# CFGpp-diffusion/CFGpp

Measured on AMD Instinct MI355X. Metric: images/sec, higher is better.
Workload: dtype fp16; 1 GPU; SD1.5 512x512 ddim_cfg++ 50 NFE lambda=0.6 batch=8/GPU; per_gpu_batch=8, global_batch=8, nfe=50, unet_batch_rows=16, weights=seeded synthetic, exact diffusers shapes, build_id=cfgpp-build:d24daf2249552bfd:nogit

## Files before the change

### cfgpp_amd/_lib.py

```python
from __future__ import annotations

import ctypes as C
import os

HERE = os.path.dirname(os.path.abspath(__file__))
LIB_PATH = os.environ.get("CFGPP_LIB") or os.path.join(HERE, "libcfgpp_hip.so")


class CfgppError(RuntimeError):
    pass


class UNetConfigC(C.Structure):
    _fields_ = [
        ("in_channels", C.c_int), ("out_channels", C.c_int),
        ("num_levels", C.c_int),
        ("block_out_channels", C.c_int * 4),
        ("layers_per_block", C.c_int),
        ("level_has_attn", C.c_int * 4),
        ("transformer_depth", C.c_int * 4),
        ("num_heads", C.c_int * 4),
        ("cross_attention_dim", C.c_int),
        ("addition_embed", C.c_int),
        ("addition_time_embed_dim", C.c_int),
        ("addition_pooled_dim", C.c_int),
        ("norm_groups", C.c_int),
        ("sample_h", C.c_int), ("sample_w", C.c_int),
        ("max_rows", C.c_int),
    ]


_P, _I, _F, _L = C.c_void_p, C.c_int, C.c_float, C.c_long

PROTOTYPES = {
    "cfgpp_last_error": (C.c_char_p, []),
    "cfgpp_build_id": (C.c_char_p, []),
    "cfgpp_step_ddim": (_I, [_P, _P, _P, _P, _I, _F, _F, _F, _F, _F, _I, _I, _L, _P]),
    "cfgpp_step_ddim_h": (_I, [_P, _P, _P, _P, _F, _F, _F, _F, _F, _I, _I, _L, _P]),
    "cfgpp_step_ddim_masked": (_I, [_P, _P, _P, _P, _F, _F, _F, _F, _F, _I, _I, _P, _P, _P, _F, _F, _I, _L, _P]),
    "cfgpp_kdiff_input": (_I, [_P, _P, _F, _I, _L, _P]),
    "cfgpp_step_kdiff": (_I, [_P, _P, _P, _P, _P, C.POINTER(C.c_float), _I, _I, _I, _I, _L, _P]),
    "cfgpp_kdiff_denoise": (_I, [_P, _P, _P, _F, _F, _P, _P, _L, _P]),
    "cfgpp_lincomb": (_I, [_P, _P, _P, _P, _F, _F, _I, _L, _P]),
    "cfgpp_unet_create": (_P, [C.POINTER(UNetConfigC), _I]),
    "cfgpp_unet_destroy": (None, [_P]),
    "cfgpp_unet_load_tensor": (_I, [_P, C.c_char_p, _P, _I, C.POINTER(C.c_long), _I]),
    "cfgpp_unet_missing": (_I, [_P]),
    "cfgpp_unet_finalize": (_I, [_P]),
    "cfgpp_unet_set_context": (_I, [_P, _P, _I, _I, _P, _P, _I, _P]),
    "cfgpp_unet_image_condition": (_I, [_P, _P, _I, _P]),
    "cfgpp_unet_forward": (_I, [_P, _P, _I, _I, _F, _P, _I, _P]),
    "cfgpp_sample_graph_ddim": (_I, [_P, _P, _P, _I, _I, _P, _P, _P, _I, C.POINTER(C.c_float), _I, _F, _I, _I, _P]),
    "cfgpp_unet_profile": (_I, [_P, _P, _I, _I, _F, _P, _I, _P, C.POINTER(C.c_double), C.POINTER(C.c_double), C.POINTER(C.c_int), C.c_char_p, _L]),
    "cfgpp_unet_tuning": (_I, [_P, _I, C.POINTER(C.c_int), _I, _I]),
    "cfgpp_unet_attach_control": (_I, [_P, _P, _F]),
    "cfgpp_unet_flops": (C.c_double, [_P, _I]),
    "cfgpp_unet_device_bytes": (C.c_double, [_P]),
    "cfgpp_vae_create": (_P, [_I, _I, _I, _F, _I]),
    "cfgpp_vae_destroy": (None, [_P]),
    "cfgpp_vae_load_tensor": (_I, [_P, C.c_char_p, _P, _I, C.POINTER(C.c_long), _I]),
    "cfgpp_vae_finalize": (_I, [_P]),
    "cfgpp_vae_decode": (_I, [_P, _P, _P, _I, _P]),
    "cfgpp_vae_decode_image": (_I, [_P, _P, _P, _I, _P]),
    "cfgpp_vae_encode": (_I, [_P, _P, _P, _P, _P, _I, _P]),
    "cfgpp_vae_profile": (_I, [_P, _P, _P, _I, _P, C.c_char_p, C.c_long]),
    "cfgpp_vae_flops": (C.c_double, [_P, _I]),
    "cfgpp_text_create": (_P, [_I, _I, _I, _I, _I, _I, _I, _I, _I]),
    "cfgpp_text_destroy": (None, [_P]),
    "cfgpp_text_load_tensor": (_I, [_P, C.c_char_p, _P, _I, C.POINTER(C.c_long), _I]),
    "cfgpp_text_finalize": (_I, [_P]),
    "cfgpp_text_encode": (_I, [_P, C.POINTER(C.c_int), C.POINTER(C.c_int), _I, _I, _P, _P, _P]),
    "cfgpp_text_device_bytes": (C.c_double, [_P]),
    "cfgpp_vae_encode_flops": (C.c_double, [_P, _I]),
    "cfgpp_vae_device_bytes": (C.c_double, [_P]),
}

DEBUG_PROTOTYPES = {
    "cfgpp_op_softmax_rows": (_I, [_P, _L, _I, _P]),
    "cfgpp_op_conv_in_ex": (_I, [_P, _I, _P, _P, _P, _I, _I, _I, _I, _I, _I, _P, _P, _F, _P]),
    "cfgpp_op_groupnorm": (_I, [_P, _P, _P, _P, _P, _P, _I, _I, _I, _I, _I, _I, _F, _I, _I, _P]),
    "cfgpp_op_groupnorm_pre": (_I, [_P, _P, _P, _P, _P, _P, _P, _P, _I, _I, _I, _I, _I, _I, _F, _I, _I, _P]),
    "cfgpp_op_igemm_set_gstat": (None, [_P]),
    "cfgpp_op_igemm_gstat_written": (_I, []),
    "cfgpp_groupnorm_set_prestats": (None, [_I]),
    "cfgpp_groupnorm_prestats_enabled": (_I, []),
    "cfgpp_op_layernorm": (_I, [_P, _P, _P, _P, _L, _I, _F, _P]),
    "cfgpp_op_attention_prepare_vt": (_I, [_P, _I, _I, _I, _P]),
    "cfgpp_op_attention": (_I, [_P, _P, _P, _P, _I, _I, _I, _I, _I, _I, _I, _P]),
    "cfgpp_op_conv_in": (_I, [_P, _I, _P, _P, _P, _I, _I, _I, _I, _I, _I, _P]),
    "cfgpp_op_conv_in_cond": (_I, [_P, _I, _P, _I, _I, _P, _P, _P, _I, _I, _I, _I, _I, _I, _P]),
    "cfgpp_op_conv_in_add": (_I, [_P, _I, _P, _I, _I, _P, _I, _P, _P, _P, _I, _I, _I, _I, _I, _I, _P]),
    "cfgpp_op_cn_conv3x3": (_I, [_P, _I, _P, _I, _P, _P, _I, _I, _I, _I, _I, _I, _I, _P]),
    "cfgpp_op_residual_add": (_I, [C.POINTER(C.c_void_p), C.POINTER(C.c_void_p), C.POINTER(C.c_int), _I, _I, _F, _P]),
    "cfgpp_op_residual_nchw": (_I, [_P, _P, _I, _I, _I, _I, _F, _P]),
    "cfgpp_controlnet_residual": (_I, [_P, _I, _F, _P, _I, C.POINTER(C.c_int), _P]),
    "cfgpp_op_vae_posterior": (_I, [_P, _P, _P, _P, _P, _P, _I, _I, _F, _P]),
    "cfgpp_op_conv_out": (_I, [_P, _P, _I, _P, _P, _I, _I, _I, _I, _I, _P]),
    "cfgpp_op_conv_out_ex": (_I, [_P, _P, _I, _P, _P, _I, _I, _I, _I, _I, _F, _F, _I, _P]),
    "cfgpp_conv_out_set_tiled": (None, [_I]),
    "cfgpp_op_sinusoid": (_I, [_P, _F, _P, _I, _I, _I, _I, _P]),
    "cfgpp_op_skinny_gemm": (_I, [_P, _I, _P, _P, _P, _I, _P, _I, _I, _I, _I, _I, _I, _P]),
    "cfgpp_op_f16_to_f32_rows": (_I, [_P, _P, _I, _I, _I, _I, _P]),
    "cfgpp_op_igemm": (_I, [_P, _P, _I, _I, _I, _I, _I, _I, _P, _I, _I, _P, _P, _I, _P, _I, _I, _P, _I, _I, _I, _P]),
    "cfgpp_op_igemm_heads": (_I, [_P, _I, _P, _I, _I, _P, _I, _P, _P, _P, _I, _I, _I, _I, _I, _I, _P]),
    "cfgpp_igemm_force_config": (None, [_I]),
    "cfgpp_igemm_set_staging": (None, [_I]),
    "cfgpp_igemm_set_staged_epilogue": (None, [_I]),
    "cfgpp_igemm_set_big_tiles": (None, [_I]),
    "cfgpp_igemm_set_tail_split": (None, [_I]),
    "cfgpp_igemm_set_autotune": (None, [_I]),
    "cfgpp_igemm_set_blocked_walk": (None, [_I]),
    "cfgpp_igemm_walk_plan_probe": (None, [_I, _I, _I, _I, _I, _I, _I, C.POINTER(C.c_int)]),
    "cfgpp_igemm_set_n_major": (None, [_I]),
    "cfgpp_igemm_force_split": (None, [_I]),
    "cfgpp_igemm_set_split_tile": (None, [_I]),
    "cfgpp_igemm_set_mf16": (None, [_I]),
    "cfgpp_igemm_set_mf16_rounds": (None, [_I]),
    "cfgpp_igemm_set_mf16_heads": (None, [_I]),
    "cfgpp_igemm_set_mf16_linear": (None, [_I]),
    "cfgpp_igemm_set_big_split": (None, [_I]),
    "cfgpp_igemm_set_tune_mask": (None, [C.c_uint]),
    "cfgpp_igemm_tuner_state": (C.c_uint, []),
    "cfgpp_igemm_timeline": (None, [_P, _L, _I]),
    "cfgpp_igemm_timeline_info": (None, [C.POINTER(C.c_int)]),
    "cfgpp_groupnorm_set_mode": (None, [_I]),
    "cfgpp_layernorm_set_rows_per_wave": (None, [_I]),
    "cfgpp_attention_set_dma": (None, [_I]),
    "cfgpp_attention_set_stagger": (None, [_I]),
    "cfgpp_attention_set_cross": (None, [_I]),
}

_lib = None


def load():
    global _lib
    if _lib is not None:
        return _lib
    if not os.path.exists(LIB_PATH):
        raise CfgppError(
            f"{LIB_PATH} not found: build it with `python -m cfgpp_amd.build` "
            "(__graft_entry__.build()).  The HIP path has no CPU fallback.")
    import torch
    try:
        lib = C.CDLL(LIB_PATH)
    except OSError as e:
        raise CfgppError(f"cannot load {LIB_PATH}: {e}") from e
    for name, (res, args) in list(PROTOTYPES.items()) + list(DEBUG_PROTOTYPES.items()):
        try:
            fn = getattr(lib, name)
        except AttributeError as e:
            raise CfgppError(f"{LIB_PATH} does not export {name}") from e
        fn.restype = res
        fn.argtypes = args
    if os.environ.get("CFGPP_AUTOTUNE", "1") == "0":
        lib.cfgpp_igemm_set_autotune(0)
    _lib = lib
    return lib


def build_id() -> str:
    return load().cfgpp_build_id().decode("utf-8", "replace")


def last_error() -> str:
    return load().cfgpp_last_error().decode("utf-8", "replace")


def check(rc: int, what: str):
    if rc != 0:
        raise CfgppError(f"{what} failed (rc={rc}): {last_error()}")
```

### cfgpp_amd/csrc/cfgpp_debug.h

```cpp
#ifndef CFGPP_DEBUG_H
#define CFGPP_DEBUG_H
#ifdef __cplusplus
extern "C" {
#endif

int cfgpp_op_softmax_rows(void* s, long rows, int ncols, void* stream);
int cfgpp_op_conv_in_ex(const void* z, int z_is_half, void* out, const float* w, const float* bias,
                        int R, int zB, int Cin, int H, int W, int Cout, const float* pre_w, const float* pre_b,
                        float in_scale, void* stream);
int cfgpp_op_groupnorm(const void* src0, const void* src1, void* dst, const float* gamma, const float* beta,
                       float* stats, int N, int H, int W, int C0, int C1, int G, float eps, int silu,
                       int dst_padded, void* stream);
int cfgpp_op_groupnorm_pre(const void* src0, const void* src1, void* dst, const float* gamma, const float* beta,
                           const float* gst0, const float* gst1, float* stats, int N, int H, int W, int C0, int C1, int G,
                           float eps, int silu, int dst_padded, void* stream);
void cfgpp_op_igemm_set_gstat(void* buf);
int cfgpp_op_igemm_gstat_written(void);
void cfgpp_groupnorm_set_prestats(int on);
int cfgpp_groupnorm_prestats_enabled(void);
void cfgpp_groupnorm_set_mode(int mode);
int cfgpp_op_layernorm(const void* x, void* y, const float* gamma, const float* beta, long rows, int C,
                       float eps, void* stream);
void cfgpp_layernorm_set_rows_per_wave(int rpw);
int cfgpp_op_attention_prepare_vt(void* vt, int BH, int d, int tok_pad, void* stream);
int cfgpp_op_attention(const void* q, const void* k, const void* vt, void* o, int B, int heads, int d,
                       int nq, int nk, int q_tok_pad, int k_tok_pad, void* stream);
void cfgpp_attention_set_dma(int mode);
void cfgpp_attention_set_stagger(int sleeps);
void cfgpp_attention_set_cross(int on);
int cfgpp_op_conv_in(const void* z, int z_is_half, void* out, const float* w, const float* bias,
                     int R, int zB, int Cin, int H, int W, int Cout, void* stream);
int cfgpp_op_conv_in_cond(const void* z, int z_is_half, const void* cond, int cond_rows, int Cc, void* out, const float* w,
                          const float* bias, int R, int zB, int Cz, int H, int W, int Cout, void* stream);
int cfgpp_op_conv_in_add(const void* z, int z_is_half, const void* cond, int cond_rows, int Cc, const void* addend, int add_rows,
                         void* out, const float* w, const float* bias, int R, int zB, int Cz, int H, int W, int Cout, void* stream);
int cfgpp_op_cn_conv3x3(const void* in, int in_kind, void* out, int out_pad, const float* w, const float* bias, int R, int Ci, int Co,
                        int Hi, int Wi, int stride, int silu, void* stream);
int cfgpp_op_residual_add(void* const* dst, const void* const* src, const int* hwc, int n, int rows, float scale, void* stream);
int cfgpp_op_residual_nchw(const void* src, float* out, int rows, int H, int W, int C, float scale, void* stream);
int cfgpp_controlnet_residual(cfgpp_unet* cn, int i, float scale, float* out, int rows, int* hwc_out, void* stream);

int cfgpp_op_vae_posterior(const float* conv_out, const float* qw, const float* qb, const float* noise, float* z,
                           float* moments, int B, int HW, float scale, void* stream);
int cfgpp_op_conv_out(const void* x, void* out, int out_is_half, const void* w, const float* bias,
                      int R, int H, int W, int C, int Cout, void* stream);
int cfgpp_op_conv_out_ex(const void* x, void* out, int out_is_half, const void* w, const float* bias,
                         int R, int H, int W, int C, int Cout, float post_scale, float post_shift, int clamp01, void* stream);
void cfgpp_conv_out_set_tiled(int on);
int cfgpp_op_sinusoid(const float* vals, float scalar, float* out, int count, int dim, int out_ld, int out_off,
                      void* stream);
int cfgpp_op_skinny_gemm(const float* x, int ldx, const void* w, const float* bias, const float* addend, int add_ld,
                         float* out, int ldo, int M, int N, int K, int silu_in, int silu_out, void* stream);
int cfgpp_op_f16_to_f32_rows(const void* in, float* out, int rows, int cols, int out_ld, int out_off, void* stream);

int cfgpp_op_igemm(const void* a0, const void* a1, int C0, int C1, int taps, int amode, int H, int W,
                   const void* w, int M, int N, const float* bias, const float* temb, int temb_ld,
                   const void* resid, int rmode, int rld, void* out, int omode, int old_, int epi,
                   void* stream);
int cfgpp_op_igemm_heads(const void* a, int K, const void* w, int M, int N, const float* bias, int rows_per_batch,
                         void* hq, void* hk, void* hvt, int part0, int part_width, int head_dim, int heads,
                         int q_tok_pad, int tok_pad, void* stream);
void cfgpp_igemm_force_config(int cfg);
void cfgpp_igemm_set_tail_split(int on);
void cfgpp_igemm_set_mf16(int mode);
void cfgpp_igemm_set_mf16_linear(int on);
void cfgpp_igemm_set_mf16_heads(int on);
void cfgpp_igemm_set_mf16_rounds(int n);
void cfgpp_igemm_set_split_tile(int cfg);
void cfgpp_igemm_force_split(int s);
void cfgpp_igemm_set_big_split(int min_kt);
void cfgpp_igemm_set_n_major(int mode);
void cfgpp_igemm_set_blocked_walk(int on);
void cfgpp_igemm_walk_plan_probe(int M, int N, int K, int BM, int BN, int smem, int n_major, int* out5);
void cfgpp_igemm_set_tune_mask(unsigned mask);
unsigned cfgpp_igemm_tuner_state(void);
void cfgpp_igemm_set_autotune(int on);
void cfgpp_igemm_set_big_tiles(int on);
void cfgpp_igemm_set_staged_epilogue(int on);
void cfgpp_igemm_set_staging(int glds);
void cfgpp_igemm_timeline(void* buf, long cap_blocks, int target);
void cfgpp_igemm_timeline_info(int* out12);

#ifdef __cplusplus
}
#endif
#endif
```

### cfgpp_amd/csrc/common.h

```cpp
#pragma once
#include <hip/hip_runtime.h>
#include <stdint.h>

typedef _Float16 half_t;
typedef _Float16 half2_t __attribute__((ext_vector_type(2)));
typedef _Float16 half4_t __attribute__((ext_vector_type(4)));
typedef _Float16 half8_t __attribute__((ext_vector_type(8)));
typedef float f32x4 __attribute__((ext_vector_type(4)));
typedef float f32x16 __attribute__((ext_vector_type(16)));

#define CFGPP_WAVE 64

void cfgpp_set_error(const char* fmt, ...);
int cfgpp_claim_device(int device_id);
#define CFGPP_HIP_CHECK(expr)                                                         \
    do {                                                                              \
        hipError_t _e = (expr);                                                       \
        if (_e != hipSuccess) {                                                       \
            cfgpp_set_error("%s:%d: %s -> %s", __FILE__, __LINE__, #expr,             \
                            hipGetErrorString(_e));                                   \
            return -1;                                                                \
        }                                                                             \
    } while (0)
#define CFGPP_REQUIRE(cond, ...)                                                      \
    do {                                                                              \
        if (!(cond)) {                                                                \
            cfgpp_set_error(__VA_ARGS__);                                             \
            return -2;                                                                \
        }                                                                             \
    } while (0)

int step_advance_launch(const float* tab, int* idx, float* cur, hipStream_t s);
int step_ddim_dev_launch(void* z, void* z0t_out, const void* eps_uc, const void* eps_c, int eps_is_half, int z_is_half, float lam,
                         const float* cdev, int tweedie_uc, int renoise_uc, long n, hipStream_t s);

struct CnAddEntry {
    half_t* dst;
    const half_t* src;
    int H, W, C, pad_;
};
int cn_residual_add_launch(const CnAddEntry* tab, int n, long max_n8, int rows, float scale, hipStream_t s);

static inline int cdiv(long a, long b) { return (int)((a + b - 1) / b); }

struct RowMap {
    int mode;
    int H, W;
    int ld;
};

__host__ __device__ __forceinline__ int cfgpp_vt_pos(int tok) {
    return (tok & ~12) | ((tok & 4) << 1) | ((tok & 8) >> 1);
}

__device__ __forceinline__ float silu_f(float x) { return x / (1.0f + __expf(-x)); }
__device__ __forceinline__ float gelu_erf_f(float x) {
    const float ax = fabsf(x) * 0.70710678118654752440f;
    const float t = __builtin_amdgcn_rcpf(1.0f + 0.3275911f * ax);
    const float poly = t * (0.254829592f + t * (-0.284496736f + t * (1.421413741f + t * (-1.453152027f + t * 1.061405429f))));
    const float erfc_ax = poly * __builtin_amdgcn_exp2f(-ax * ax * 1.4426950408889634f);
    const float cdf = x >= 0.f ? 1.0f - 0.5f * erfc_ax : 0.5f * erfc_ax;
    return x * cdf;
}

typedef float f32x2 __attribute__((ext_vector_type(2)));
#define CFGPP_GELU_C 4.75f
#define CFGPP_GELU_POLY {4.912262559e-01f, 5.645360425e-02f, -1.591939032e-01f, 2.464362979e-01f, -1.982378513e-01f, 1.363233291e-02f, \
                         1.386516690e-01f, -1.158297956e-01f, -9.092462249e-03f, 6.090912968e-02f, -1.936562732e-02f, -1.160200126e-02f, \
                         6.012340542e-03f}
__device__ __forceinline__ f32x2 gelu_erf_pk(f32x2 x) {
    constexpr float k[13] = CFGPP_GELU_POLY;
    f32x2 a;
    a.x = fminf(fabsf(x.x), CFGPP_GELU_C); a.y = fminf(fabsf(x.y), CFGPP_GELU_C);
    const f32x2 t = __builtin_elementwise_fma(a, (f32x2){2.0f / CFGPP_GELU_C, 2.0f / CFGPP_GELU_C}, (f32x2){-1.0f, -1.0f});
    f32x2 p = {k[12], k[12]};
#pragma unroll
    for (int i = 11; i >= 0; --i) p = __builtin_elementwise_fma(p, t, (f32x2){k[i], k[i]});
    f32x2 m;
    m.x = fabsf(x.x) * p.x; m.y = fabsf(x.y) * p.y;
    return __builtin_elementwise_fma(x, (f32x2){0.5f, 0.5f}, m);
}

template <int MAXV>
__device__ __forceinline__ void ln_row_stats(const half8_t (&raw)[MAXV], int chunks, int C, float eps, int lane,
                                             float (&v)[MAXV][8], float& mean, float& rstd) {
    float sum = 0.f;
#pragma unroll
    for (int j = 0; j < MAXV; ++j) {
        const bool live = lane + j * 64 < chunks;
#pragma unroll
        for (int k = 0; k < 8; ++k) { v[j][k] = live ? (float)raw[j][k] : 0.f; sum += v[j][k]; }
    }
#pragma unroll
    for (int o = 32; o > 0; o >>= 1) sum += __shfl_xor(sum, o);
    mean = sum / (float)C;
    float sq = 0.f;
#pragma unroll
    for (int j = 0; j < MAXV; ++j) {
        const bool live = lane + j * 64 < chunks;
#pragma unroll
        for (int k = 0; k < 8; ++k) { const float d = v[j][k] - mean; sq += live ? d * d : 0.f; }
    }
#pragma unroll
    for (int o = 32; o > 0; o >>= 1) sq += __shfl_xor(sq, o);
    rstd = rsqrtf(sq / (float)C + eps);
}
__device__ __forceinline__ half8_t ln_row_affine(const float (&v)[8], float mean, float rstd, const float4 (&g)[2], const float4 (&be)[2]) {
    const float gg[8] = {g[0].x, g[0].y, g[0].z, g[0].w, g[1].x, g[1].y, g[1].z, g[1].w};
    const float bb[8] = {be[0].x, be[0].y, be[0].z, be[0].w, be[1].x, be[1].y, be[1].z, be[1].w};
    half8_t o;
#pragma unroll
    for (int k = 0; k < 8; ++k) o[k] = (half_t)((v[k] - mean) * rstd * gg[k] + bb[k]);
    return o;
}
```

### cfgpp_amd/csrc/engine_base.h

```cpp
#pragma once
#include <algorithm>
#include <cmath>
#include <cstring>
#include <deque>
#include <functional>
#include <map>
#include <string>
#include <vector>

#include "../../include/cfgpp.h"
#include "cfgpp_debug.h"
#include "igemm.h"

namespace {


struct HostParam {
    std::vector<long> shape;
    std::vector<half_t> h;
    std::vector<float> f;
    bool is_matrix = false;
    bool loaded = false;
    long numel() const { long n = 1; for (long s : shape) n *= s; return n; }
};

struct Tensor {
    half_t* p = nullptr;
    int H = 0, W = 0, C = 0;
    float* gst = nullptr;
    int* gst_ok = nullptr;
};

using Op = std::function<int(hipStream_t, int )>;


struct EngineBase {
    int max_rows = 1;
    int norm_groups = 32;
    std::map<std::string, HostParam> params;
    std::vector<void*> allocs;
    double dev_bytes = 0;
    double macs_per_row = 0;
    double attn_macs_per_row = 0;

    std::vector<Op> plan;
    std::vector<int> plan_kind;
    std::vector<double> plan_macs;
    std::vector<std::string> plan_desc;
    void tag(int kind, double macs, const std::string& desc = "") {
        plan_kind.resize(plan.size(), 3); plan_macs.resize(plan.size(), 0.0); plan_desc.resize(plan.size());
        if (!plan.empty()) { plan_kind.back() = kind; plan_macs.back() = macs; plan_desc.back() = desc; }
    }
    std::deque<int> cfg_hints;
    std::vector<int*> plan_hint;
    int tuned_rows = 0;
    std::map<int, std::vector<int>> tuned_by_rows;
    int* new_hint(bool in_main_plan) {
        cfg_hints.push_back(0);
        int* h = &cfg_hints.back();
        if (in_main_plan) { plan_hint.resize(plan.size() + 1, nullptr); plan_hint[plan.size()] = h; }
        return h;
    }
    int tune_plan(hipStream_t s, int rows) {
        auto cached = tuned_by_rows.find(rows);
        if (cached != tuned_by_rows.end() && cached->second.size() == cfg_hints.size()) {
            size_t k = 0;
            for (int& h : cfg_hints) h = cached->second[k++];
            tuned_rows = rows;
            return 0;
        }
        static const int cands[] = {0, 1, 4, 5, 6, 7, 8, 9, 10, 11, 12, 13, 14, 15, 16, 17, 20, 24, 25, 26, 27, 28};
        const size_t n = plan.size();
        plan_hint.resize(n, nullptr);
        hipStreamCaptureStatus cap = hipStreamCaptureStatusNone;
        if (hipStreamIsCapturing(s, &cap) != hipSuccess || cap != hipStreamCaptureStatusNone) return 0;
        std::vector<hipEvent_t> ev(n + 1, nullptr);
        for (auto& e : ev) if (hipEventCreate(&e) != hipSuccess) return -1;
        std::vector<float> base(n, 1e30f), best(n, 1e30f), t(n);
        std::vector<char> applied(n, 1);
        std::vector<int> bestc(n, 0);
        int rc = 0;
        auto timed_passes = [&]() {
            std::fill(t.begin(), t.end(), 1e30f);
            for (int rep = 0; rep < 2 && rc == 0; ++rep) {
                if (hipEventRecord(ev[0], s) != hipSuccess) rc = -1;
                for (size_t i = 0; i < n && rc == 0; ++i) {
                    rc = plan[i](s, rows);
                    if (plan_hint[i]) applied[i] = (char)igemm_last_hint_applied();
                    if (rc == 0 && hipEventRecord(ev[i + 1], s) != hipSuccess) rc = -1;
                }
                if (rc == 0 && hipEventSynchronize(ev[n]) != hipSuccess) rc = -1;
                for (size_t i = 0; i < n && rc == 0; ++i) {
                    if (!plan_hint[i]) continue;
                    float ms = 0.f;
                    if (hipEventElapsedTime(&ms, ev[i], ev[i + 1]) == hipSuccess && ms < t[i]) t[i] = ms;
                }
            }
        };
        const unsigned mask = igemm_tune_mask();
        for (int c : cands) {
            if (c != 0 && !((mask >> c) & 1u)) continue;
            for (int& h : cfg_hints) h = c;
            timed_passes();
            for (size_t i = 0; i < n; ++i) {
                if (c == 0) base[i] = t[i];
                if (t[i] < best[i] && (c == 0 || applied[i])) { best[i] = t[i]; bestc[i] = c; }
            }
        }
        for (size_t i = 0; i < n; ++i)
            if (plan_hint[i] && !(bestc[i] != 0 && best[i] < 0.97f * base[i])) { bestc[i] = 0; best[i] = base[i]; }
        for (int walk = 1; walk <= 2 && rc == 0 && (mask >> 31); ++walk) {
            for (size_t i = 0; i < n; ++i) if (plan_hint[i]) *plan_hint[i] = (bestc[i] & 63) | (walk << 6);
            timed_passes();
            for (size_t i = 0; i < n; ++i)
                if (plan_hint[i] && t[i] < 0.97f * best[i]) { best[i] = t[i]; bestc[i] = (bestc[i] & 63) | (walk << 6); }
        }
        for (int& h : cfg_hints) h = 0;
        for (size_t i = 0; i < n; ++i) if (plan_hint[i]) *plan_hint[i] = bestc[i];
        for (auto& e : ev) hipEventDestroy(e);
        if (rc == 0) tuned_by_rows[rows] = std::vector<int>(cfg_hints.begin(), cfg_hints.end());
        tuned_rows = rows;
        return rc;
    }
    std::map<std::tuple<int, int, int>, std::vector<std::pair<half_t*, float*>>> pool;
    std::deque<int> gst_flags;
    float* d_gn_stats = nullptr;
    static constexpr long KSPLIT_WS_BYTES = 128L << 20;
    float* d_ksplit_ws = nullptr;
    float* ksplit_ws() {
        if (!d_ksplit_ws) d_ksplit_ws = (float*)dmalloc((size_t)KSPLIT_WS_BYTES, false);
        return d_ksplit_ws;
    }

    void* dmalloc(size_t bytes, bool zero = true) {
        void* p = nullptr;
        if (hipMalloc(&p, bytes) != hipSuccess) return nullptr;
        if (zero) hipMemset(p, 0, bytes);
        allocs.push_back(p);
        dev_bytes += (double)bytes;
        return p;
    }
    Tensor acq(int H, int W, int C) {
        auto key = std::make_tuple(H, W, C);
        auto& fl = pool[key];
        Tensor t; t.H = H; t.W = W; t.C = C;
        gst_flags.push_back(0);
        t.gst_ok = &gst_flags.back();
        if (!fl.empty()) { t.p = fl.back().first; t.gst = fl.back().second; fl.pop_back(); return t; }
        t.p = (half_t*)dmalloc((size_t)max_rows * (H + 2) * (W + 2) * C * sizeof(half_t));
        if (H * W >= 1024 && (H * W) % 32 == 0 && C % 8 == 0)
            t.gst = (float*)dmalloc((size_t)max_rows * (H * W / 32) * C * 2 * sizeof(float), false);
        return t;
    }
    void rel(const Tensor& t) { if (t.p) pool[std::make_tuple(t.H, t.W, t.C)].push_back(std::make_pair(t.p, t.gst)); }
    ~EngineBase() { for (void* p : allocs) hipFree(p); }
};

void expect(EngineBase* u, const std::string& key, std::vector<long> shape, bool matrix) {
    HostParam hp; hp.shape = std::move(shape); hp.is_matrix = matrix;
    u->params[key] = std::move(hp);
}
void expect_linear(EngineBase* u, const std::string& p, long out, long in, bool bias = true) {
    expect(u, p + ".weight", {out, in}, true);
    if (bias) expect(u, p + ".bias", {out}, false);
}
void expect_conv(EngineBase* u, const std::string& p, long out, long in, int k) {
    expect(u, p + ".weight", {out, in, k, k}, true);
    expect(u, p + ".bias", {out}, false);
}
void expect_norm(EngineBase* u, const std::string& p, long c) {
    expect(u, p + ".weight", {c}, false);
    expect(u, p + ".bias", {c}, false);
}
void expect_resnet(EngineBase* u, const std::string& p, long cin, long cout, long temb) {
    expect_norm(u, p + ".norm1", cin);
    expect_conv(u, p + ".conv1", cout, cin, 3);
    expect_linear(u, p + ".time_emb_proj", cout, temb);
    expect_norm(u, p + ".norm2", cout);
    expect_conv(u, p + ".conv2", cout, cout, 3);
    if (cin != cout) expect_conv(u, p + ".conv_shortcut", cout, cin, 1);
}
void expect_transformer(EngineBase* u, const std::string& p, long c, int depth, long cross) {
    expect_norm(u, p + ".norm", c);
    expect(u, p + ".proj_in.weight", {c, c}, true);  expect(u, p + ".proj_in.bias", {c}, false);
    expect(u, p + ".proj_out.weight", {c, c}, true); expect(u, p + ".proj_out.bias", {c}, false);
    for (int k = 0; k < depth; ++k) {
        const std::string b = p + ".transformer_blocks." + std::to_string(k);
        expect_norm(u, b + ".norm1", c); expect_norm(u, b + ".norm2", c); expect_norm(u, b + ".norm3", c);
        expect_linear(u, b + ".attn1.to_q", c, c, false); expect_linear(u, b + ".attn1.to_k", c, c, false);
        expect_linear(u, b + ".attn1.to_v", c, c, false); expect_linear(u, b + ".attn1.to_out.0", c, c, true);
        expect_linear(u, b + ".attn2.to_q", c, c, false); expect_linear(u, b + ".attn2.to_k", c, cross, false);
        expect_linear(u, b + ".attn2.to_v", c, cross, false); expect_linear(u, b + ".attn2.to_out.0", c, c, true);
        expect_linear(u, b + ".ff.net.0.proj", 8 * c, c, true);
        expect_linear(u, b + ".ff.net.2", c, 4 * c, true);
    }
}

struct Builder {
    EngineBase* u;
    bool ok = true;
    std::string err;

    HostParam* get(const std::string& key) {
        auto it = u->params.find(key);
        if (it == u->params.end() || !it->second.loaded) { ok = false; err = "missing parameter " + key; return nullptr; }
        return &it->second;
    }
    template <typename T>
    T* upload(const std::vector<T>& v) {
        T* d = (T*)u->dmalloc(v.size() * sizeof(T), false);
        if (!d) { ok = false; err = "hipMalloc failed"; return nullptr; }
        if (hipMemcpy(d, v.data(), v.size() * sizeof(T), hipMemcpyHostToDevice) != hipSuccess) { ok = false; err = "hipMemcpy failed"; }
        return d;
    }
    void drop(const std::string& key) { auto& p = u->params[key]; std::vector<half_t>().swap(p.h); std::vector<float>().swap(p.f); }

    float* f32(const std::string& key) {
        HostParam* p = get(key); if (!p) return nullptr;
        float* d = upload(p->f); drop(key); return d;
    }
    half_t* linear(const std::string& key) {
        HostParam* p = get(key); if (!p) return nullptr;
        half_t* d = upload(p->h); drop(key); return d;
    }
    half_t* conv3(const std::string& key) {
        HostParam* p = get(key); if (!p) return nullptr;
        const long O = p->shape[0], I = p->shape[1];
        std::vector<half_t> r((size_t)O * 9 * I);
        for (long o = 0; o < O; ++o)
            for (long i = 0; i < I; ++i)
                for (int t = 0; t < 9; ++t) r[(size_t)o * 9 * I + ((i >> 6) * 9 + t) * 64 + (i & 63)] = p->h[((size_t)o * I + i) * 9 + t];
        half_t* d = upload(r); drop(key); return d;
    }
    std::vector<half_t> concat_host(const std::vector<std::string>& keys) {
        std::vector<half_t> r;
        for (auto& k : keys) { HostParam* p = get(k); if (!p) return {}; r.insert(r.end(), p->h.begin(), p->h.end()); }
        for (auto& k : keys) drop(k);
        return r;
    }
    half_t* concat(const std::vector<std::string>& keys) {
        std::vector<half_t> r = concat_host(keys);
        return ok ? upload(r) : nullptr;
    }
    bool geglu_host(const std::string& pfx, long C, std::vector<half_t>& rw, std::vector<float>& rb) {
        HostParam* pw = get(pfx + ".weight"); HostParam* pb = get(pfx + ".bias");
        if (!pw || !pb) return false;
        const long F = 4 * C;
        rw.resize((size_t)2 * F * C); rb.resize((size_t)2 * F);
        for (long f = 0; f < F; ++f) {
            const long pv = (f / 32) * 64 + (f % 32), pg = pv + 32;
            std::memcpy(&rw[(size_t)pv * C], &pw->h[(size_t)f * C], C * sizeof(half_t));
            std::memcpy(&rw[(size_t)pg * C], &pw->h[(size_t)(F + f) * C], C * sizeof(half_t));
            rb[pv] = pb->f[f]; rb[pg] = pb->f[F + f];
        }
        drop(pfx + ".weight"); drop(pfx + ".bias");
        return true;
    }
    void geglu(const std::string& pfx, long C, half_t** w, float** b) {
        std::vector<half_t> rw; std::vector<float> rb;
        if (!geglu_host(pfx, C, rw, rb)) return;
        *w = upload(rw); *b = upload(rb);
    }
};

inline int round_up(int a, int b) { return (a + b - 1) / b * b; }

IGemmArgs base_args(EngineBase* u = nullptr) {
    IGemmArgs a; std::memset(&a, 0, sizeof(a)); a.out_scale = 1.0f; a.taps = 1;
    if (u) { a.ws_buf = u->ksplit_ws(); a.ws_bytes = a.ws_buf ? EngineBase::KSPLIT_WS_BYTES : 0; }
    return a;
}

struct Plan {
    EngineBase* u;
    Builder* B;
    std::vector<Op>* ops;

    void conv3x3(const Tensor& src, const Tensor& dst, const half_t* w, const float* bias, int amode,
                 const float* temb, int temb_ld, const Tensor* resid, int ashift = 0) {
        IGemmArgs a = base_args(u);
        a.a0 = src.p; a.C0 = src.C; a.taps = 9; a.amode = amode; a.ashift = ashift; a.H = dst.H; a.W = dst.W;
        a.w = w; a.N = dst.C; a.K = 9 * src.C; a.bias = bias; a.temb = temb; a.temb_ld = temb_ld;
        a.rows_per_batch = dst.H * dst.W;
        if (resid) { a.resid = resid->p; a.rmode = 1; a.rld = resid->C; }
        a.out = dst.p; a.omode = 1; a.old = dst.C; a.epi = EPI_STORE;
        a.gstat = dst.gst; a.stat_flag = dst.gst ? dst.gst_ok : nullptr;
        const int HW = dst.H * dst.W;
        u->macs_per_row += (double)HW * dst.C * 9.0 * src.C;
        int* hint = u->new_hint(ops == &u->plan);
        ops->push_back([a, HW, hint](hipStream_t s, int rows) mutable { IGemmArgs b = a; b.M = rows * HW; b.cfg_hint = *hint; return igemm_launch(b, s); });
        if (ops == &u->plan) u->tag(0, (double)HW * dst.C * 9.0 * src.C, "conv3x3 amode=" + std::to_string(amode) + " HW=" + std::to_string(HW) + " N=" + std::to_string(dst.C) + " K=" + std::to_string(9 * src.C) + (resid ? " +res" : "") + (temb ? " +temb" : ""));
    }
    void conv1x1(const Tensor& s0, const Tensor* s1, const Tensor& dst, const half_t* w, const float* bias) {
        IGemmArgs a = base_args(u);
        a.a0 = s0.p; a.C0 = s0.C; if (s1) { a.a1 = s1->p; a.C1 = s1->C; }
        a.amode = 1; a.H = dst.H; a.W = dst.W; a.w = w; a.N = dst.C; a.K = a.C0 + a.C1; a.bias = bias;
        a.rows_per_batch = dst.H * dst.W; a.out = dst.p; a.omode = 1; a.old = dst.C; a.epi = EPI_STORE;
        const int HW = dst.H * dst.W;
        u->macs_per_row += (double)HW * dst.C * a.K;
        int* hint = u->new_hint(ops == &u->plan);
        ops->push_back([a, HW, hint](hipStream_t s, int rows) mutable { IGemmArgs b = a; b.M = rows * HW; b.cfg_hint = *hint; return igemm_launch(b, s); });
        if (ops == &u->plan) u->tag(0, (double)HW * dst.C * a.K, "conv1x1 HW=" + std::to_string(HW) + " N=" + std::to_string(dst.C) + " K=" + std::to_string(a.K));
    }
    void linear(const half_t* A, int K, half_t* out, int N, const half_t* w, const float* bias, const half_t* resid,
                int tokens, int epi = EPI_STORE) {
        IGemmArgs a = base_args(u);
        a.a0 = A; a.C0 = K; a.amode = 0; a.w = w; a.N = N; a.K = K; a.bias = bias;
        a.resid = resid; a.rmode = 0; a.rld = N; a.out = out; a.omode = 0;
        a.old = (epi == EPI_GEGLU) ? N / 2 : N; a.epi = epi; a.rows_per_batch = tokens;
        u->macs_per_row += (double)tokens * N * K;
        int* hint = u->new_hint(ops == &u->plan);
        ops->push_back([a, tokens, hint](hipStream_t s, int rows) mutable { IGemmArgs b = a; b.M = rows * tokens; b.cfg_hint = *hint; return igemm_launch(b, s); });
        if (ops == &u->plan) u->tag(0, (double)tokens * N * K, std::string(epi == EPI_GEGLU ? "geglu" : "linear") + " HW=" + std::to_string(tokens) + " N=" + std::to_string(N) + " K=" + std::to_string(K) + (resid ? " +res" : ""));
    }
    void linear_to_padded(const half_t* A, int K, const Tensor& dst, const half_t* w, const float* bias, const Tensor& resid) {
        IGemmArgs a = base_args(u);
        a.a0 = A; a.C0 = K; a.amode = 0; a.H = dst.H; a.W = dst.W; a.w = w; a.N = dst.C; a.K = K; a.bias = bias;
        a.resid = resid.p; a.rmode = 1; a.rld = resid.C; a.out = dst.p; a.omode = 1; a.old = dst.C;
        a.epi = EPI_STORE; a.rows_per_batch = dst.H * dst.W;
        a.gstat = dst.gst; a.stat_flag = dst.gst ? dst.gst_ok : nullptr;
        const int HW = dst.H * dst.W;
        u->macs_per_row += (double)HW * dst.C * K;
        int* hint = u->new_hint(ops == &u->plan);
        ops->push_back([a, HW, hint](hipStream_t s, int rows) mutable { IGemmArgs b = a; b.M = rows * HW; b.cfg_hint = *hint; return igemm_launch(b, s); });
        if (ops == &u->plan) u->tag(0, (double)HW * dst.C * K, "proj_out HW=" + std::to_string(HW) + " N=" + std::to_string(dst.C) + " K=" + std::to_string(K));
    }
    void heads(const half_t* A, int K, const half_t* w, int N, int tokens, int part0, int C, int nheads,
               half_t* q, half_t* k, half_t* vt, int q_tok_pad, int tok_pad, bool count = true,
               const float* bias = nullptr) {
        IGemmArgs a = base_args(u);
        const int d = C / nheads;
        a.a0 = A; a.C0 = K; a.amode = 0; a.w = w; a.N = N; a.K = K; a.epi = EPI_HEADS;
        a.bias = bias;
        a.rows_per_batch = tokens; a.hq = q; a.hk = k; a.hvt = vt; a.part0 = part0; a.part_width = C;
        a.head_dim = d; a.head_dim_pad = round_up(d, 32); a.heads = nheads; a.tok_pad = tok_pad; a.q_tok_pad = q_tok_pad;
        if (count) u->macs_per_row += (double)tokens * N * K;
        int* hint = u->new_hint(ops == &u->plan);
        ops->push_back([a, tokens, hint](hipStream_t s, int rows) mutable { IGemmArgs b = a; b.M = rows * tokens; b.cfg_hint = *hint; return igemm_launch(b, s); });
        if (ops == &u->plan) u->tag(0, count ? (double)tokens * N * K : 0.0, "heads HW=" + std::to_string(tokens) + " N=" + std::to_string(N) + " K=" + std::to_string(K));
    }
    void groupnorm(const Tensor& s0, const Tensor* s1, half_t* dst, bool dst_padded, const float* g, const float* b,
                   float eps, bool silu) {
        EngineBase* uu = u;
        const half_t* p0 = s0.p; const half_t* p1 = s1 ? s1->p : nullptr;
        const int H = s0.H, W = s0.W, C0 = s0.C, C1 = s1 ? s1->C : 0, G = u->norm_groups;
        const float* gst0 = s0.gst; const float* gst1 = s1 ? s1->gst : nullptr;
        const int* ok0 = s0.gst_ok; const int* ok1 = s1 ? s1->gst_ok : nullptr;
        ops->push_back([=](hipStream_t s, int rows) {
            if (cfgpp_groupnorm_prestats_enabled() && gst0 && ok0 && *ok0 && (!p1 || (gst1 && ok1 && *ok1)))
                return cfgpp_op_groupnorm_pre(p0, p1, dst, g, b, gst0, gst1, uu->d_gn_stats, rows, H, W, C0, C1, G, eps, silu ? 1 : 0,
                                              dst_padded ? 1 : 0, s);
            return cfgpp_op_groupnorm(p0, p1, dst, g, b, uu->d_gn_stats, rows, H, W, C0, C1, G, eps, silu ? 1 : 0,
                                      dst_padded ? 1 : 0, s);
        });
        if (ops == &u->plan) u->tag(2, 0.0, "groupnorm HW=" + std::to_string(H * W) + " C=" + std::to_string(C0 + C1));
    }
    void layernorm(const half_t* x, half_t* y, const float* g, const float* b, int tokens, int C) {
        ops->push_back([=](hipStream_t s, int rows) { return cfgpp_op_layernorm(x, y, g, b, (long)rows * tokens, C, 1e-5f, s); });
        if (ops == &u->plan) u->tag(2, 0.0, "layernorm HW=" + std::to_string(tokens) + " C=" + std::to_string(C));
    }
    void attention(const half_t* q, const half_t* k, const half_t* vt, half_t* o, int nheads, int d, int nq, int nk,
                   int q_tok_pad, int k_tok_pad) {
        u->attn_macs_per_row += 2.0 * (double)nheads * nq * nk * d;
        ops->push_back([=](hipStream_t s, int rows) {
            return cfgpp_op_attention(q, k, vt, o, rows, nheads, d, nq, nk, q_tok_pad, k_tok_pad, s);
        });
        if (ops == &u->plan) u->tag(1, 2.0 * (double)nheads * nq * nk * d, "self_attn heads=" + std::to_string(nheads) + " N=" + std::to_string(nq) + " d=" + std::to_string(d));
    }
};

}
```

### cfgpp_amd/csrc/small_kernels.hip

```cpp
#include "common.h"

namespace {

template <typename TIN>
__global__ void __launch_bounds__(256)
conv_in_kernel(const TIN* __restrict__ z, const half_t* __restrict__ cond, int Cc, int cond_rows,
               half_t* __restrict__ out, const float* __restrict__ w,
               const float* __restrict__ bias, int R, int zB, int Cz, int H, int W, int Cout,
               const float* __restrict__ pre_w, const float* __restrict__ pre_b, float in_scale,
               const half_t* __restrict__ add, int add_rows) {
    constexpr int TP = 16;
    __shared__ float patch[TP][9 * 16];
    const int r = blockIdx.y;
    const int p0 = blockIdx.x * TP;
    const int HW = H * W;
    const int zb = r % zB;
    const int cb = cond ? zb % cond_rows : 0;
    const int Cin = Cz + Cc;
    const int K = 9 * Cin;
    for (int i = threadIdx.x; i < TP * K; i += blockDim.x) {
        const int tp = i / K, k = i - tp * K;
        const int tap = k / Cin, ci = k - tap * Cin;
        const int p = p0 + tp;
        float v = 0.f;
        if (p < HW) {
            const int y = p / W + tap / 3 - 1, x = p % W + tap % 3 - 1;
            if (y >= 0 && y < H && x >= 0 && x < W) {
                if (ci >= Cz) {
                    v = (float)cond[((long)(cb * Cc + ci - Cz) * H + y) * W + x];
                } else if (pre_w) {
                    float acc = pre_b ? pre_b[ci] : 0.f;
                    for (int j = 0; j < Cz; ++j)
                        acc += pre_w[ci * Cz + j] * (float)(half_t)((float)z[((long)(zb * Cz + j) * H + y) * W + x] * in_scale);
                    v = acc;
                } else {
                    v = (float)z[((long)(zb * Cz + ci) * H + y) * W + x] * in_scale;
                }
            }
        }
        patch[tp][k] = (float)(half_t)v;
    }
    __syncthreads();
    for (int co = threadIdx.x; co < Cout; co += blockDim.x) {
        float acc[TP];
        const float b = bias ? bias[co] : 0.f;
#pragma unroll
        for (int tp = 0; tp < TP; ++tp) acc[tp] = b;
        for (int k = 0; k < K; ++k) {
            const float wv = w[(long)k * Cout + co];
#pragma unroll
            for (int tp = 0; tp < TP; ++tp) acc[tp] += wv * patch[tp][k];
        }
#pragma unroll
        for (int tp = 0; tp < TP; ++tp) {
            const int p = p0 + tp;
            if (p < HW) {
                const int y = p / W, x = p - y * W;
                half_t v = (half_t)acc[tp];
                if (add) v = (half_t)((float)v + (float)add[((long)((zb % add_rows) * (H + 2) + y + 1) * (W + 2) + x + 1) * Cout + co]);
                out[((long)(r * (H + 2) + y + 1) * (W + 2) + x + 1) * Cout + co] = v;
            }
        }
    }
}

template <int CO, typename TOUT>
__global__ void __launch_bounds__(256)
conv_out_kernel(const half_t* __restrict__ x, TOUT* __restrict__ out, const half_t* __restrict__ w,
                const float* __restrict__ bias, int R, int H, int W, int C, int cout_real,
                float post_scale, float post_shift, int clamp01) {
    const int lane = threadIdx.x & 63;
    const long pix = (long)blockIdx.x * 4 + (threadIdx.x >> 6);
    const long total = (long)R * H * W;
    if (pix >= total) return;
    const int HW = H * W;
    const int r = (int)(pix / HW), p = (int)(pix - (long)r * HW);
    const int y = p / W, xq = p - y * W;
    const int cpt = C / 8;
    float acc[CO];
#pragma unroll
    for (int o = 0; o < CO; ++o) acc[o] = 0.f;
    for (int c = lane; c < 9 * cpt; c += 64) {
        const int tap = c / cpt, cc = (c - tap * cpt) * 8;
        const int dy = tap / 3 - 1, dx = tap % 3 - 1;
        const half8_t xv = *reinterpret_cast<const half8_t*>(
            x + ((long)(r * (H + 2) + y + 1 + dy) * (W + 2) + xq + 1 + dx) * C + cc);
#pragma unroll
        for (int o = 0; o < CO; ++o) {
            const half8_t wv = *reinterpret_cast<const half8_t*>(w + ((long)o * 9 + tap) * C + cc);
#pragma unroll
            for (int k = 0; k < 8; ++k) acc[o] += (float)xv[k] * (float)wv[k];
        }
    }
#pragma unroll
    for (int o = 0; o < CO; ++o)
#pragma unroll
        for (int s = 32; s > 0; s >>= 1) acc[o] += __shfl_xor(acc[o], s);
    if (lane < cout_real) {
        float v = 0.f;
#pragma unroll
        for (int o = 0; o < CO; ++o) if (lane == o) v = acc[o];
        v += bias ? bias[lane] : 0.f;
        v = v * post_scale + post_shift;
        if (clamp01) v = fminf(fmaxf(v, 0.f), 1.f);
        out[((long)(r * cout_real + lane) * H + y) * W + xq] = (TOUT)v;
    }
}

template <int CO, typename TOUT>
__global__ void __launch_bounds__(256)
conv_out_tile_kernel(const half_t* __restrict__ x, TOUT* __restrict__ out, const half_t* __restrict__ w,
                     const float* __restrict__ bias, int R, int H, int W, int C, int cout_real,
                     float post_scale, float post_shift, int clamp01) {
    constexpr int TH = 8, TW = 32, HH = TH + 2, HW_ = TW + 2, PITCH = 144;
    __shared__ __attribute__((aligned(16))) char tile[HH * HW_ * PITCH];
    const int tid = threadIdx.x;
    const int tiles_x = (W + TW - 1) / TW, tiles_y = (H + TH - 1) / TH;
    int b = blockIdx.x;
    const int txi = b % tiles_x; b /= tiles_x;
    const int tyi = b % tiles_y; const int r = b / tiles_y;
    const int y0 = tyi * TH, x0 = txi * TW;
    const int ty = tid >> 5, tx = tid & 31;
    typedef _Float16 h2 __attribute__((ext_vector_type(2)));
    float acc[CO];
#pragma unroll
    for (int o = 0; o < CO; ++o) acc[o] = 0.f;
    const half_t* xr = x + (long)r * (H + 2) * (W + 2) * C;
    for (int cb = 0; cb < C; cb += 64) {
        __syncthreads();
        for (int i = tid; i < HH * HW_ * 8; i += 256) {
            const int px = i >> 3, ch = i & 7;
            const int hy = px / HW_, hx = px - hy * HW_;
            const int gy = y0 + hy, gx = x0 + hx;
            half8_t v = {0, 0, 0, 0, 0, 0, 0, 0};
            if (gy < H + 2 && gx < W + 2) v = *reinterpret_cast<const half8_t*>(xr + ((long)gy * (W + 2) + gx) * C + cb + ch * 8);
            *reinterpret_cast<half8_t*>(tile + px * PITCH + ch * 16) = v;
        }
        __syncthreads();
#pragma unroll
        for (int tap = 0; tap < 9; ++tap) {
            const int dy = tap / 3, dx = tap - 3 * (tap / 3);
            const char* px = tile + ((ty + dy) * HW_ + tx + dx) * PITCH;
#pragma unroll
            for (int ch = 0; ch < 8; ++ch) {
                const half8_t xv = *reinterpret_cast<const half8_t*>(px + ch * 16);
#pragma unroll
                for (int o = 0; o < CO; ++o) {
                    const half8_t wv = *reinterpret_cast<const half8_t*>(w + ((long)o * 9 + tap) * C + cb + ch * 8);
#pragma unroll
                    for (int k = 0; k < 4; ++k)
                        acc[o] = __builtin_amdgcn_fdot2((h2){xv[2 * k], xv[2 * k + 1]}, (h2){wv[2 * k], wv[2 * k + 1]}, acc[o], false);
                }
            }
        }
    }
    const int y = y0 + ty, xq = x0 + tx;
    if (y < H && xq < W) {
#pragma unroll
        for (int o = 0; o < CO; ++o) {
            if (o < cout_real) {
                float v = acc[o] + (bias ? bias[o] : 0.f);
                v = v * post_scale + post_shift;
                if (clamp01) v = fminf(fmaxf(v, 0.f), 1.f);
                out[((long)(r * cout_real + o) * H + y) * W + xq] = (TOUT)v;
            }
        }
    }
}

__global__ void sinusoid_kernel(const float* __restrict__ vals, float scalar, float* __restrict__ out,
                                int count, int dim, int out_ld, int out_off) {
    const int i = blockIdx.x;
    const int half_dim = dim / 2;
    const float v = vals ? vals[i] : scalar;
    for (int j = threadIdx.x; j < half_dim; j += blockDim.x) {
        const float e = expf(-9.210340371976184f * (float)j / (float)half_dim);
        const float arg = v * e;
        out[(long)i * out_ld + out_off + j] = (float)(half_t)cosf(arg);
        out[(long)i * out_ld + out_off + half_dim + j] = (float)(half_t)sinf(arg);
    }
}

template <int MB, int NB>
__global__ void __launch_bounds__(256)
skinny_gemm_kernel(const float* __restrict__ x, int ldx, const half_t* __restrict__ w, const float* __restrict__ bias,
                   const float* __restrict__ addend, int add_ld, float* __restrict__ out, int ldo,
                   int M, int N, int K, int silu_in, int silu_out) {
    const int lane = threadIdx.x & 63, wid = threadIdx.x >> 6;
    const int n0 = (blockIdx.x * 4 + wid) * NB;
    const int m0 = blockIdx.y * MB;
    if (n0 >= N) return;
    float acc[MB][NB];
#pragma unroll
    for (int i = 0; i < MB; ++i)
#pragma unroll
        for (int j = 0; j < NB; ++j) acc[i][j] = 0.f;
    for (int kc = lane * 8; kc < K; kc += 64 * 8) {
        float xv[MB][8];
#pragma unroll
        for (int i = 0; i < MB; ++i) {
            const int m = min(m0 + i, M - 1);
            const float4 a = *reinterpret_cast<const float4*>(x + (long)m * ldx + kc);
            const float4 b = *reinterpret_cast<const float4*>(x + (long)m * ldx + kc + 4);
            xv[i][0] = a.x; xv[i][1] = a.y; xv[i][2] = a.z; xv[i][3] = a.w;
            xv[i][4] = b.x; xv[i][5] = b.y; xv[i][6] = b.z; xv[i][7] = b.w;
            if (silu_in) {
#pragma unroll
                for (int k = 0; k < 8; ++k) xv[i][k] = silu_f(xv[i][k]);
            }
        }
#pragma unroll
        for (int j = 0; j < NB; ++j) {
            const int n = min(n0 + j, N - 1);
            const half8_t wv = *reinterpret_cast<const half8_t*>(w + (long)n * K + kc);
#pragma unroll
            for (int i = 0; i < MB; ++i)
#pragma unroll
                for (int k = 0; k < 8; ++k) acc[i][j] += xv[i][k] * (float)wv[k];
        }
    }
#pragma unroll
    for (int i = 0; i < MB; ++i)
#pragma unroll
        for (int j = 0; j < NB; ++j)
#pragma unroll
            for (int s = 32; s > 0; s >>= 1) acc[i][j] += __shfl_xor(acc[i][j], s);
    if (lane == 0) {
#pragma unroll
        for (int i = 0; i < MB; ++i) {
            const int m = m0 + i;
            if (m >= M) continue;
#pragma unroll
            for (int j = 0; j < NB; ++j) {
                const int n = n0 + j;
                if (n >= N) continue;
                float v = acc[i][j] + (bias ? bias[n] : 0.f);
                if (addend) v += addend[(long)m * add_ld + n];
                if (silu_out) v = silu_f(v);
                out[(long)m * ldo + n] = v;
            }
        }
    }
}

__global__ void f16_to_f32_rows_kernel(const half_t* __restrict__ in, float* __restrict__ out, int rows, int cols,
                                       int out_ld, int out_off) {
    const long n = (long)rows * cols;
    for (long i = (long)blockIdx.x * blockDim.x + threadIdx.x; i < n; i += (long)gridDim.x * blockDim.x) {
        const int r = (int)(i / cols), c = (int)(i - (long)r * cols);
        out[(long)r * out_ld + out_off + c] = (float)in[i];
    }
}

}


__global__ void __launch_bounds__(256)
vae_posterior_kernel(const float* __restrict__ co, const float* __restrict__ qw, const float* __restrict__ qb,
                     const float* __restrict__ noise, float* __restrict__ z, float* __restrict__ moments,
                     int B, int HW, float scale) {
    const long i = (long)blockIdx.x * blockDim.x + threadIdx.x;
    if (i >= (long)B * HW) return;
    const int b = (int)(i / HW), p = (int)(i - (long)b * HW);
    float x[8], m[8];
#pragma unroll
    for (int j = 0; j < 8; ++j) x[j] = (float)(half_t)co[((long)b * 8 + j) * HW + p];
#pragma unroll
    for (int o = 0; o < 8; ++o) {
        float acc = qb[o];
#pragma unroll
        for (int j = 0; j < 8; ++j) acc += qw[o * 8 + j] * x[j];
        m[o] = (float)(half_t)acc;
    }
#pragma unroll
    for (int c = 0; c < 4; ++c) {
        const float lv = fminf(fmaxf(m[4 + c], -30.f), 20.f);
        const float n = noise ? noise[((long)b * 4 + c) * HW + p] : 0.f;
        z[((long)b * 4 + c) * HW + p] = (m[c] + __expf(0.5f * lv) * n) * scale;
        if (moments) { moments[((long)b * 8 + c) * HW + p] = m[c]; moments[((long)b * 8 + 4 + c) * HW + p] = lv; }
    }
}

extern "C" {

int cfgpp_op_vae_posterior(const float* conv_out, const float* qw, const float* qb, const float* noise, float* z,
                           float* moments, int B, int HW, float scale, void* stream) {
    CFGPP_REQUIRE(conv_out && qw && qb && z && B > 0 && HW > 0, "vae_posterior: bad args");
    hipLaunchKernelGGL(vae_posterior_kernel, dim3(cdiv((long)B * HW, 256)), dim3(256), 0, (hipStream_t)stream, conv_out, qw, qb, noise, z, moments, B, HW, scale);
    CFGPP_HIP_CHECK(hipGetLastError());
    return 0;
}

int cfgpp_op_conv_in_add(const void* z, int z_is_half, const void* cond, int cond_rows, int Cc, const void* addend, int add_rows,
                         void* out, const float* w, const float* bias, int R, int zB, int Cz, int H, int W, int Cout, void* stream);

int cfgpp_op_conv_in_cond(const void* z, int z_is_half, const void* cond, int cond_rows, int Cc, void* out, const float* w,
                          const float* bias, int R, int zB, int Cz, int H, int W, int Cout, void* stream) {
    return cfgpp_op_conv_in_add(z, z_is_half, cond, cond_rows, Cc, nullptr, 1, out, w, bias, R, zB, Cz, H, W, Cout, stream);
}

int cfgpp_op_conv_in_add(const void* z, int z_is_half, const void* cond, int cond_rows, int Cc, const void* addend, int add_rows,
                         void* out, const float* w, const float* bias, int R, int zB, int Cz, int H, int W, int Cout, void* stream) {
    CFGPP_REQUIRE(Cz >= 1 && Cz <= 8, "conv_in: Cin=%d (<= 8)", Cz);
    CFGPP_REQUIRE(!addend || add_rows > 0, "conv_in: addend with add_rows=%d", add_rows);
    const half_t* add = (const half_t*)addend;
    if (!add) add_rows = 1;
    CFGPP_REQUIRE(!cond || (Cc >= 1 && Cz + Cc <= 16 && cond_rows > 0), "conv_in: condition of %d channels x %d rows on %d latent channels (Cin <= 16)",
                  Cc, cond_rows, Cz);
    CFGPP_REQUIRE(z && out && w && R > 0 && zB > 0, "conv_in: bad args");
    if (!cond) { Cc = 0; cond_rows = 1; }
    dim3 grid(cdiv((long)H * W, 16), R);
    hipStream_t s = (hipStream_t)stream;
    if (z_is_half)
        hipLaunchKernelGGL(conv_in_kernel<half_t>, grid, dim3(256), 0, s, (const half_t*)z, (const half_t*)cond, Cc, cond_rows, (half_t*)out, w, bias,
                           R, zB, Cz, H, W, Cout, (const float*)nullptr, (const float*)nullptr, 1.0f, add, add_rows);
    else
        hipLaunchKernelGGL(conv_in_kernel<float>, grid, dim3(256), 0, s, (const float*)z, (const half_t*)cond, Cc, cond_rows, (half_t*)out, w, bias,
                           R, zB, Cz, H, W, Cout, (const float*)nullptr, (const float*)nullptr, 1.0f, add, add_rows);
    CFGPP_HIP_CHECK(hipGetLastError());
    return 0;
}

int cfgpp_op_conv_in_ex(const void* z, int z_is_half, void* out, const float* w, const float* bias,
                        int R, int zB, int Cin, int H, int W, int Cout, const float* pre_w, const float* pre_b,
                        float in_scale, void* stream) {
    CFGPP_REQUIRE(Cin >= 1 && Cin <= 8, "conv_in: Cin=%d (<= 8)", Cin);
    CFGPP_REQUIRE(z && out && w && R > 0 && zB > 0, "conv_in: bad args");
    dim3 grid(cdiv((long)H * W, 16), R);
    hipStream_t s = (hipStream_t)stream;
    if (z_is_half)
        hipLaunchKernelGGL(conv_in_kernel<half_t>, grid, dim3(256), 0, s, (const half_t*)z, (const half_t*)nullptr, 0, 1, (half_t*)out, w, bias,
                           R, zB, Cin, H, W, Cout, pre_w, pre_b, in_scale, (const half_t*)nullptr, 1);
    else
        hipLaunchKernelGGL(conv_in_kernel<float>, grid, dim3(256), 0, s, (const float*)z, (const half_t*)nullptr, 0, 1, (half_t*)out, w, bias,
                           R, zB, Cin, H, W, Cout, pre_w, pre_b, in_scale, (const half_t*)nullptr, 1);
    CFGPP_HIP_CHECK(hipGetLastError());
    return 0;
}

int cfgpp_op_conv_in(const void* z, int z_is_half, void* out, const float* w, const float* bias,
                     int R, int zB, int Cin, int H, int W, int Cout, void* stream) {
    return cfgpp_op_conv_in_ex(z, z_is_half, out, w, bias, R, zB, Cin, H, W, Cout, nullptr, nullptr, 1.0f, stream);
}

int cfgpp_op_conv_out_ex(const void* x, void* out, int out_is_half, const void* w, const float* bias,
                         int R, int H, int W, int C, int Cout, float post_scale, float post_shift, int clamp01, void* stream);
static int g_conv_out_tiled = 1;
void cfgpp_conv_out_set_tiled(int on) { g_conv_out_tiled = on ? 1 : 0; }

int cfgpp_op_conv_out(const void* x, void* out, int out_is_half, const void* w, const float* bias,
                      int R, int H, int W, int C, int Cout, void* stream) {
    return cfgpp_op_conv_out_ex(x, out, out_is_half, w, bias, R, H, W, C, Cout, 1.0f, 0.0f, 0, stream);
}

int cfgpp_op_conv_out_ex(const void* x, void* out, int out_is_half, const void* w, const float* bias,
                         int R, int H, int W, int C, int Cout, float post_scale, float post_shift, int clamp01, void* stream) {
    CFGPP_REQUIRE(Cout >= 1 && Cout <= 8 && C % 8 == 0, "conv_out: Cout=%d C=%d", Cout, C);
    CFGPP_REQUIRE(x && out && w, "conv_out: null pointer");
    const long total = (long)R * H * W;
    dim3 grid(cdiv(total, 4));
    hipStream_t s = (hipStream_t)stream;
    if (Cout <= 4 && C % 64 == 0 && (long)H * W >= 128 * 128 && g_conv_out_tiled) {
        dim3 tg((unsigned)((long)R * cdiv(H, 8) * cdiv(W, 32)));
        if (out_is_half)
            hipLaunchKernelGGL((conv_out_tile_kernel<4, half_t>), tg, dim3(256), 0, s, (const half_t*)x, (half_t*)out, (const half_t*)w, bias, R, H, W, C, Cout, post_scale, post_shift, clamp01);
        else if (Cout <= 3)
            hipLaunchKernelGGL((conv_out_tile_kernel<3, float>), tg, dim3(256), 0, s, (const half_t*)x, (float*)out, (const half_t*)w, bias, R, H, W, C, Cout, post_scale, post_shift, clamp01);
        else
            hipLaunchKernelGGL((conv_out_tile_kernel<4, float>), tg, dim3(256), 0, s, (const half_t*)x, (float*)out, (const half_t*)w, bias, R, H, W, C, Cout, post_scale, post_shift, clamp01);
        CFGPP_HIP_CHECK(hipGetLastError());
        return 0;
    }
    if (Cout > 4) {
        CFGPP_REQUIRE(!out_is_half, "conv_out: 8-channel output is fp32 only");
        hipLaunchKernelGGL((conv_out_kernel<8, float>), grid, dim3(256), 0, s, (const half_t*)x, (float*)out, (const half_t*)w, bias, R, H, W, C, Cout, post_scale, post_shift, clamp01);
    } else if (out_is_half)
        hipLaunchKernelGGL((conv_out_kernel<4, half_t>), grid, dim3(256), 0, s, (const half_t*)x, (half_t*)out, (const half_t*)w, bias, R, H, W, C, Cout, post_scale, post_shift, clamp01);
    else
        hipLaunchKernelGGL((conv_out_kernel<4, float>), grid, dim3(256), 0, s, (const half_t*)x, (float*)out, (const half_t*)w, bias, R, H, W, C, Cout, post_scale, post_shift, clamp01);
    CFGPP_HIP_CHECK(hipGetLastError());
    return 0;
}

int cfgpp_op_sinusoid(const float* vals, float scalar, float* out, int count, int dim, int out_ld, int out_off,
                      void* stream) {
    CFGPP_REQUIRE(out && count > 0 && dim % 2 == 0, "sinusoid: bad args");
    hipLaunchKernelGGL(sinusoid_kernel, dim3(count), dim3(128), 0, (hipStream_t)stream, vals, scalar, out, count, dim, out_ld, out_off);
    CFGPP_HIP_CHECK(hipGetLastError());
    return 0;
}

int cfgpp_op_skinny_gemm(const float* x, int ldx, const void* w, const float* bias, const float* addend, int add_ld,
                         float* out, int ldo, int M, int N, int K, int silu_in, int silu_out, void* stream) {
    CFGPP_REQUIRE(x && w && out && M > 0 && N > 0 && K % 8 == 0, "skinny_gemm: bad args (K=%d)", K);
    hipStream_t s = (hipStream_t)stream;
    if (M == 1) {
        dim3 grid(cdiv(N, 4 * 2), 1);
        hipLaunchKernelGGL((skinny_gemm_kernel<1, 2>), grid, dim3(256), 0, s, x, ldx, (const half_t*)w, bias, addend, add_ld, out, ldo, M, N, K, silu_in, silu_out);
    } else {
        dim3 grid(cdiv(N, 4 * 2), cdiv(M, 4));
        hipLaunchKernelGGL((skinny_gemm_kernel<4, 2>), grid, dim3(256), 0, s, x, ldx, (const half_t*)w, bias, addend, add_ld, out, ldo, M, N, K, silu_in, silu_out);
    }
    CFGPP_HIP_CHECK(hipGetLastError());
    return 0;
}

int cfgpp_op_f16_to_f32_rows(const void* in, float* out, int rows, int cols, int out_ld, int out_off, void* stream) {
    hipLaunchKernelGGL(f16_to_f32_rows_kernel, dim3(cdiv((long)rows * cols, 256) > 1024 ? 1024 : cdiv((long)rows * cols, 256)),
                       dim3(256), 0, (hipStream_t)stream, (const half_t*)in, out, rows, cols, out_ld, out_off);
    CFGPP_HIP_CHECK(hipGetLastError());
    return 0;
}

}
```

### cfgpp_amd/csrc/unet.hip

```cpp
#include "engine_base.h"

struct cfgpp_unet : EngineBase {
    cfgpp_unet_config cfg;
    int device = 0;
    bool finalized = false;

    std::vector<Op> ctx_plan;
    const void* in_z = nullptr; int in_z_half = 0; int in_z_rows = 0; float in_t = 0.f; void* out_eps = nullptr;
    const float* in_t_dev = nullptr;
    half_t* d_cond = nullptr; int cond_rows = 0;
    float* d_step_tab = nullptr; int step_tab_cap = 0; float* d_step_cur = nullptr; int* d_step_idx = nullptr;
    hipStream_t cap_stream = nullptr;
    struct GraphKey { const void* z; void* z0t; void* eps; const void* euc; const void* ec; int z_half, z_rows, rows, tw, rn; float lam; long n; int tuned_serial; int cond_rows; };
    struct Graph { GraphKey key; hipGraph_t graph; hipGraphExec_t exec; };
    std::vector<Graph> graphs;
    int tuned_serial = 0;
    static void destroy(Graph& g) { if (g.exec) hipGraphExecDestroy(g.exec); if (g.graph) hipGraphDestroy(g.graph); g.exec = nullptr; g.graph = nullptr; }
    void drop_graphs() { for (auto& g : graphs) destroy(g); graphs.clear(); }
    ~cfgpp_unet() { drop_graphs(); if (cap_stream) hipStreamDestroy(cap_stream); }
    const half_t* ctx_ehs = nullptr; int ctx_rows = 0; int ctx_tokens = 77;
    const half_t* ctx_text = nullptr; const float* ctx_tids = nullptr; int ctx_cond_rows = 0;
    bool ctx_set = false;

    float* d_sin_t = nullptr; float* d_emb_h = nullptr; float* d_emb_t = nullptr; float* d_emb = nullptr;
    float* d_temb_all = nullptr; int temb_total = 0;
    float* d_add_in = nullptr; float* d_add_h = nullptr; float* d_aug = nullptr;

    half_t *tok_x = nullptr, *tok_ln = nullptr, *tok_attn = nullptr, *tok_ff = nullptr;
    half_t *hq[4] = {nullptr, nullptr, nullptr, nullptr}, *hk[4] = {nullptr, nullptr, nullptr, nullptr},
           *hvt[4] = {nullptr, nullptr, nullptr, nullptr};

    bool control = false;
    std::vector<int> embed_ch;
    std::vector<Op> img_plan;
    const void* img_in = nullptr; int img_in_half = 0;
    half_t* d_img_emb = nullptr; int img_rows = 0;
    std::vector<Tensor> ctrl_res;
    std::vector<Tensor> ctrl_dst;
    cfgpp_unet* ctrl = nullptr; float ctrl_scale = 0.f;
    CnAddEntry* d_ctrl_tab = nullptr; long ctrl_max_n8 = 0;
};

namespace {

void build_param_table(cfgpp_unet* u) {
    const cfgpp_unet_config& c = u->cfg;
    const int L = c.num_levels;
    const long c0 = c.block_out_channels[0], temb = 4 * c0;
    expect_conv(u, "conv_in", c0, c.in_channels, 3);
    expect_linear(u, "time_embedding.linear_1", temb, c0);
    expect_linear(u, "time_embedding.linear_2", temb, temb);
    if (c.addition_embed) {
        const long in = (long)c.addition_time_embed_dim * 6 + c.addition_pooled_dim;
        expect_linear(u, "add_embedding.linear_1", temb, in);
        expect_linear(u, "add_embedding.linear_2", temb, temb);
    }
    long ch = c0;
    for (int i = 0; i < L; ++i) {
        const long co = c.block_out_channels[i];
        const std::string p = "down_blocks." + std::to_string(i);
        for (int j = 0; j < c.layers_per_block; ++j) {
            expect_resnet(u, p + ".resnets." + std::to_string(j), ch, co, temb);
            if (c.level_has_attn[i])
                expect_transformer(u, p + ".attentions." + std::to_string(j), co, c.transformer_depth[i], c.cross_attention_dim);
            ch = co;
        }
        if (i != L - 1) expect_conv(u, p + ".downsamplers.0.conv", co, co, 3);
    }
    const long cm = c.block_out_channels[L - 1];
    expect_resnet(u, "mid_block.resnets.0", cm, cm, temb);
    expect_transformer(u, "mid_block.attentions.0", cm, c.transformer_depth[L - 1], c.cross_attention_dim);
    expect_resnet(u, "mid_block.resnets.1", cm, cm, temb);
    if (u->control) {
        const std::vector<int>& e = u->embed_ch;
        const std::string q = "controlnet_cond_embedding.";
        expect_conv(u, q + "conv_in", e[0], 3, 3);
        for (size_t i = 0; i + 1 < e.size(); ++i) {
            expect_conv(u, q + "blocks." + std::to_string(2 * i), e[i], e[i], 3);
            expect_conv(u, q + "blocks." + std::to_string(2 * i + 1), e[i + 1], e[i], 3);
        }
        expect_conv(u, q + "conv_out", c0, e.back(), 3);
        int k = 0;
        expect_conv(u, "controlnet_down_blocks." + std::to_string(k++), c0, c0, 1);
        for (int i = 0; i < L; ++i) {
            const long co = c.block_out_channels[i];
            for (int j = 0; j < c.layers_per_block; ++j) expect_conv(u, "controlnet_down_blocks." + std::to_string(k++), co, co, 1);
            if (i != L - 1) expect_conv(u, "controlnet_down_blocks." + std::to_string(k++), co, co, 1);
        }
        expect_conv(u, "controlnet_mid_block", cm, cm, 1);
        return;
    }
    long prev = cm;
    for (int i = 0; i < L; ++i) {
        const int lvl = L - 1 - i;
        const long co = c.block_out_channels[lvl];
        const long cin_lvl = c.block_out_channels[std::max(lvl - 1, 0)];
        const std::string p = "up_blocks." + std::to_string(i);
        for (int j = 0; j < c.layers_per_block + 1; ++j) {
            const long skip = (j == c.layers_per_block) ? cin_lvl : co;
            const long rin = (j == 0 ? prev : co) + skip;
            expect_resnet(u, p + ".resnets." + std::to_string(j), rin, co, temb);
            if (c.level_has_attn[lvl])
                expect_transformer(u, p + ".attentions." + std::to_string(j), co, c.transformer_depth[lvl], c.cross_attention_dim);
        }
        if (i != L - 1) expect_conv(u, p + ".upsamplers.0.conv", co, co, 3);
        prev = co;
    }
    expect_norm(u, "conv_norm_out", c0);
    expect_conv(u, "conv_out", c.out_channels, c0, 3);
}

struct ResW {
    float *n1g, *n1b, *n2g, *n2b, *b1, *b2, *bsc;
    half_t *w1, *w2, *wsc;
    int temb_off;
    int cin, cout;
};

int controlnet_tail(cfgpp_unet* u, Builder& B, Plan& P, const std::vector<Tensor>& skips, const Tensor& mid) {
    const cfgpp_unet_config& c = u->cfg;
    const int R = c.max_rows, c0 = c.block_out_channels[0];
    auto persist = [&](int H, int W, int C) {
        Tensor t; t.H = H; t.W = W; t.C = C;
        t.p = (half_t*)u->dmalloc((size_t)R * (H + 2) * (W + 2) * C * sizeof(half_t));
        return t;
    };
    for (size_t k = 0; k <= skips.size(); ++k) {
        const Tensor& src = k < skips.size() ? skips[k] : mid;
        const std::string key = k < skips.size() ? "controlnet_down_blocks." + std::to_string(k) : std::string("controlnet_mid_block");
        half_t* w = B.linear(key + ".weight"); float* b = B.f32(key + ".bias");
        Tensor r = persist(src.H, src.W, src.C);
        CFGPP_REQUIRE(r.p, "finalize: hipMalloc failed");
        P.conv1x1(src, nullptr, r, w, b);
        u->ctrl_res.push_back(r);
    }
    const std::vector<int>& e = u->embed_ch;
    const int n = (int)e.size();
    const std::string q = "controlnet_cond_embedding.";
    struct Layer { std::string key; int ci, co, stride; };
    std::vector<Layer> layers;
    layers.push_back({q + "conv_in", 3, e[0], 1});
    for (int i = 0; i + 1 < n; ++i) {
        layers.push_back({q + "blocks." + std::to_string(2 * i), e[i], e[i], 1});
        layers.push_back({q + "blocks." + std::to_string(2 * i + 1), e[i], e[i + 1], 2});
    }
    long scratch = 1;
    {
        int h = c.sample_h << (n - 1), w = c.sample_w << (n - 1);
        for (size_t l = 0; l + 1 < layers.size(); ++l) {
            if (layers[l].stride == 2) { h = (h - 1) / 2 + 1; w = (w - 1) / 2 + 1; }
            scratch = std::max(scratch, (long)R * h * w * layers[l].co);
        }
    }
    half_t* buf[2] = {(half_t*)u->dmalloc((size_t)scratch * sizeof(half_t), false), (half_t*)u->dmalloc((size_t)scratch * sizeof(half_t), false)};
    Tensor pre = persist(c.sample_h, c.sample_w, e.back());
    CFGPP_REQUIRE(buf[0] && buf[1] && pre.p, "finalize: hipMalloc failed");
    cfgpp_unet* uu = u;
    int h = c.sample_h << (n - 1), w = c.sample_w << (n - 1);
    for (size_t l = 0; l < layers.size(); ++l) {
        const Layer& ly = layers[l];
        HostParam* pw = B.get(ly.key + ".weight");
        CFGPP_REQUIRE(pw, "finalize: %s", B.err.c_str());
        std::vector<float> r((size_t)9 * ly.ci * ly.co);
        for (int o = 0; o < ly.co; ++o) for (int i = 0; i < ly.ci; ++i) for (int t = 0; t < 9; ++t)
            r[((size_t)t * ly.ci + i) * ly.co + o] = (float)pw->h[((size_t)o * ly.ci + i) * 9 + t];
        B.drop(ly.key + ".weight");
        float* dw = B.upload(r); float* db = B.f32(ly.key + ".bias");
        const bool last = l + 1 == layers.size();
        const half_t* in = l == 0 ? nullptr : buf[(l - 1) & 1];
        half_t* out = last ? pre.p : buf[l & 1];
        const int hi = h, wi = w, ci = ly.ci, co = ly.co, st = ly.stride, first = l == 0;
        u->img_plan.push_back([=](hipStream_t s, int rows) {
            return cfgpp_op_cn_conv3x3(first ? uu->img_in : in, first ? (uu->img_in_half ? 1 : 2) : 0, out, last ? 1 : 0, dw, db, rows, ci,
                                       co, hi, wi, st, 1, s);
        });
        if (st == 2) { h = (h - 1) / 2 + 1; w = (w - 1) / 2 + 1; }
    }
    CFGPP_REQUIRE(h == c.sample_h && w == c.sample_w, "finalize: internal error, the embedding ends at %d x %d", h, w);
    {
        half_t* wo = B.conv3(q + "conv_out.weight"); float* bo = B.f32(q + "conv_out.bias");
        Tensor dst; dst.p = u->d_img_emb; dst.H = c.sample_h; dst.W = c.sample_w; dst.C = c0;
        Plan PI{u, &B, &u->img_plan};
        const double macs = u->macs_per_row;
        PI.conv3x3(pre, dst, wo, bo, 1, nullptr, 0, nullptr);
        u->macs_per_row = macs;
    }
    CFGPP_REQUIRE(B.ok, "finalize: %s", B.err.c_str());
    return 0;
}

}

extern "C" {

static cfgpp_unet* unet_new(const cfgpp_unet_config* cfg, int device_id, const int* embed, int n_embed) {
    if (!cfg) { cfgpp_set_error("unet_create: null config"); return nullptr; }
    if (cfg->num_levels < 1 || cfg->num_levels > 4 || cfg->layers_per_block < 1 || cfg->max_rows < 1) {
        cfgpp_set_error("unet_create: bad config"); return nullptr;
    }
    for (int i = 0; i < cfg->num_levels; ++i) {
        const int c = cfg->block_out_channels[i];
        if (c % 64 != 0 || c % cfg->norm_groups != 0) { cfgpp_set_error("unet_create: channels %d must be a multiple of 64 and of norm_groups", c); return nullptr; }
        if (cfg->level_has_attn[i]) {
            const int d = c / cfg->num_heads[i];
            if (c % cfg->num_heads[i] != 0 || d % 4 != 0 || d > 160) { cfgpp_set_error("unet_create: head dim %d unsupported", d); return nullptr; }
        }
    }
    if (cfg->cross_attention_dim % 64 != 0) { cfgpp_set_error("unet_create: cross_attention_dim must be a multiple of 64"); return nullptr; }
    if (!embed && cfg->in_channels > cfg->out_channels && cfg->in_channels > 16) {
        cfgpp_set_error("unet_create: in_channels=%d out_channels=%d (an inpaint UNet takes at most 16 input channels)", cfg->in_channels,
                        cfg->out_channels);
        return nullptr;
    }
    if ((cfg->sample_h % (1 << (cfg->num_levels - 1))) || (cfg->sample_w % (1 << (cfg->num_levels - 1)))) {
        cfgpp_set_error("unet_create: sample size must be divisible by 2^(levels-1)"); return nullptr;
    }
    int ndev = 0;
    if (hipGetDeviceCount(&ndev) != hipSuccess || ndev <= device_id) {
        cfgpp_set_error("unet_create: no HIP device %d (found %d) - the HIP path has no CPU fallback", device_id, ndev);
        return nullptr;
    }
    if (cfgpp_claim_device(device_id)) return nullptr;
    if (hipSetDevice(device_id) != hipSuccess) { cfgpp_set_error("unet_create: hipSetDevice failed"); return nullptr; }
    cfgpp_unet* u = new cfgpp_unet();
    u->cfg = *cfg; u->device = device_id; u->max_rows = cfg->max_rows; u->norm_groups = cfg->norm_groups;
    if (embed) { u->control = true; u->embed_ch.assign(embed, embed + n_embed); }
    build_param_table(u);
    return u;
}

cfgpp_unet* cfgpp_unet_create(const cfgpp_unet_config* cfg, int device_id) {
    if (cfg && cfg->out_channels == 0) {
        static const int embed[4] = {16, 32, 96, 256};
        if (cfg->in_channels < 1 || cfg->in_channels > 8) {
            cfgpp_set_error("unet_create: ControlNet (out_channels = 0) with in_channels=%d (1 .. 8 latent channels)", cfg->in_channels);
            return nullptr;
        }
        return unet_new(cfg, device_id, embed, 4);
    }
    return unet_new(cfg, device_id, nullptr, 0);
}


void cfgpp_unet_destroy(cfgpp_unet* u) {
    if (!u) return;
    delete u;
}

int cfgpp_unet_load_tensor(cfgpp_unet* u, const char* key, const void* host, int dtype, const long* shape, int ndim) {
    CFGPP_REQUIRE(u && key && host && shape, "load_tensor: null argument");
    CFGPP_REQUIRE(!u->finalized, "load_tensor: context already finalized");
    auto it = u->params.find(key);
    if (it == u->params.end()) { cfgpp_set_error("load_tensor: unknown key %s", key); return -3; }
    HostParam& p = it->second;
    long n = 1; for (int i = 0; i < ndim; ++i) n *= shape[i];
    CFGPP_REQUIRE(n == p.numel(), "load_tensor: %s has %ld elements, expected %ld", key, n, p.numel());
    if (ndim == 4) { p.shape.assign(shape, shape + 4); }
    if (p.is_matrix && !(std::string(key) == "conv_in.weight")) {
        p.h.resize(n);
        if (dtype == 0) { const float* s = (const float*)host; for (long i = 0; i < n; ++i) p.h[i] = (half_t)s[i]; }
        else std::memcpy(p.h.data(), host, n * sizeof(half_t));
    } else {
        p.f.resize(n);
        if (dtype == 0) std::memcpy(p.f.data(), host, n * sizeof(float));
        else { const half_t* s = (const half_t*)host; for (long i = 0; i < n; ++i) p.f[i] = (float)s[i]; }
    }
    p.loaded = true;
    return 0;
}

int cfgpp_unet_missing(cfgpp_unet* u) {
    if (!u) return -1;
    int n = 0; std::string names;
    for (auto& kv : u->params) if (!kv.second.loaded) { if (n < 8) names += kv.first + " "; ++n; }
    if (n) cfgpp_set_error("missing %d parameters: %s...", n, names.c_str());
    return n;
}

int cfgpp_unet_finalize(cfgpp_unet* u) {
    CFGPP_REQUIRE(u, "finalize: null");
    CFGPP_REQUIRE(!u->finalized, "finalize: already finalized");
    if (cfgpp_unet_missing(u) != 0) { const std::string m = cfgpp_last_error(); cfgpp_set_error("finalize: %s", m.c_str()); return -2; }
    CFGPP_HIP_CHECK(hipSetDevice(u->device));
    const cfgpp_unet_config& c = u->cfg;
    const int L = c.num_levels, R = c.max_rows;
    const int c0 = c.block_out_channels[0], temb_dim = 4 * c0;
    Builder B{u};
    Plan P{u, &B, &u->plan};
    Plan PC{u, &B, &u->ctx_plan};

    long max_tok_c = 0, max_ff = 0;
    {
        int H = c.sample_h, W = c.sample_w;
        for (int i = 0; i < L; ++i) {
            const long C = c.block_out_channels[i];
            if (c.level_has_attn[i] || i == L - 1) {
                const long tok = (long)H * W;
                const int d = (int)(C / c.num_heads[i]), dp = round_up(d, 32);
                max_tok_c = std::max(max_tok_c, tok * C);
                max_ff = std::max(max_ff, tok * 4 * C);
                u->hq[i] = (half_t*)u->dmalloc((size_t)R * c.num_heads[i] * round_up((int)tok, 128) * dp * 2);
                u->hk[i] = (half_t*)u->dmalloc((size_t)R * c.num_heads[i] * round_up((int)tok, 128) * dp * 2);
                u->hvt[i] = (half_t*)u->dmalloc((size_t)R * c.num_heads[i] * dp * round_up((int)tok, 64) * 2);
                CFGPP_REQUIRE(u->hq[i] && u->hk[i] && u->hvt[i], "finalize: hipMalloc failed");
                if (cfgpp_op_attention_prepare_vt(u->hvt[i], R * c.num_heads[i], d, round_up((int)tok, 64), nullptr)) return -1;
            }
            if (i != L - 1) { H /= 2; W /= 2; }
        }
    }
    u->tok_x = (half_t*)u->dmalloc((size_t)R * max_tok_c * 2);
    u->tok_ln = (half_t*)u->dmalloc((size_t)R * max_tok_c * 2);
    u->tok_attn = (half_t*)u->dmalloc((size_t)R * max_tok_c * 2);
    u->tok_ff = (half_t*)u->dmalloc((size_t)R * max_ff * 2);
    u->d_gn_stats = (float*)u->dmalloc((size_t)R * (1024 * 64 * 2 + 64 * 2) * sizeof(float));
    u->d_sin_t = (float*)u->dmalloc((size_t)c0 * sizeof(float));
    u->d_emb_h = (float*)u->dmalloc((size_t)temb_dim * sizeof(float));
    u->d_emb_t = (float*)u->dmalloc((size_t)temb_dim * sizeof(float));
    u->d_emb = (float*)u->dmalloc((size_t)R * temb_dim * sizeof(float));
    CFGPP_REQUIRE(u->tok_x && u->tok_ln && u->tok_attn && u->tok_ff, "finalize: hipMalloc failed");

    std::vector<std::string> res_names;
    {
        for (int i = 0; i < L; ++i)
            for (int j = 0; j < c.layers_per_block; ++j) res_names.push_back("down_blocks." + std::to_string(i) + ".resnets." + std::to_string(j));
        res_names.push_back("mid_block.resnets.0"); res_names.push_back("mid_block.resnets.1");
        for (int i = 0; i < L && !u->control; ++i)
            for (int j = 0; j < c.layers_per_block + 1; ++j) res_names.push_back("up_blocks." + std::to_string(i) + ".resnets." + std::to_string(j));
    }
    std::map<std::string, int> temb_off;
    half_t* w_temb_all = nullptr; float* b_temb_all = nullptr;
    {
        std::vector<half_t> wa; std::vector<float> ba; int off = 0;
        for (auto& rn : res_names) {
            HostParam* pw = B.get(rn + ".time_emb_proj.weight"); HostParam* pb = B.get(rn + ".time_emb_proj.bias");
            CFGPP_REQUIRE(pw && pb, "finalize: %s", B.err.c_str());
            temb_off[rn] = off; off += (int)pw->shape[0];
            wa.insert(wa.end(), pw->h.begin(), pw->h.end()); ba.insert(ba.end(), pb->f.begin(), pb->f.end());
            B.drop(rn + ".time_emb_proj.weight"); B.drop(rn + ".time_emb_proj.bias");
        }
        u->temb_total = off;
        w_temb_all = B.upload(wa); b_temb_all = B.upload(ba);
        u->d_temb_all = (float*)u->dmalloc((size_t)R * off * sizeof(float));
    }
    const bool per_row_temb = c.addition_embed != 0;
    const int temb_ld = per_row_temb ? u->temb_total : 0;

    {
        half_t* w1 = B.linear("time_embedding.linear_1.weight"); float* b1 = B.f32("time_embedding.linear_1.bias");
        half_t* w2 = B.linear("time_embedding.linear_2.weight"); float* b2 = B.f32("time_embedding.linear_2.bias");
        cfgpp_unet* uu = u;
        u->plan.push_back([=](hipStream_t s, int) { return cfgpp_op_sinusoid(uu->in_t_dev, uu->in_t, uu->d_sin_t, 1, c0, c0, 0, s); });
        u->plan.push_back([=](hipStream_t s, int) { return cfgpp_op_skinny_gemm(uu->d_sin_t, c0, w1, b1, nullptr, 0, uu->d_emb_h, temb_dim, 1, temb_dim, c0, 0, 1, s); });
        if (per_row_temb) {
            u->plan.push_back([=](hipStream_t s, int rows) {
                const int add_ld = uu->ctx_cond_rows == 1 ? 0 : temb_dim;
                return cfgpp_op_skinny_gemm(uu->d_emb_h, 0, w2, b2, uu->d_aug, add_ld, uu->d_emb, temb_dim, rows, temb_dim, temb_dim, 0, 0, s);
            });
            u->plan.push_back([=](hipStream_t s, int rows) {
                return cfgpp_op_skinny_gemm(uu->d_emb, temb_dim, w_temb_all, b_temb_all, nullptr, 0, uu->d_temb_all, uu->temb_total, rows, uu->temb_total, temb_dim, 1, 0, s);
            });
        } else {
            u->plan.push_back([=](hipStream_t s, int) { return cfgpp_op_skinny_gemm(uu->d_emb_h, temb_dim, w2, b2, nullptr, 0, uu->d_emb_t, temb_dim, 1, temb_dim, temb_dim, 0, 0, s); });
            u->plan.push_back([=](hipStream_t s, int) {
                return cfgpp_op_skinny_gemm(uu->d_emb_t, temb_dim, w_temb_all, b_temb_all, nullptr, 0, uu->d_temb_all, uu->temb_total, 1, uu->temb_total, temb_dim, 1, 0, s);
            });
        }
        if (c.addition_embed) {
            const int tdim = c.addition_time_embed_dim, pooled = c.addition_pooled_dim, in = 6 * tdim + pooled;
            half_t* aw1 = B.linear("add_embedding.linear_1.weight"); float* ab1 = B.f32("add_embedding.linear_1.bias");
            half_t* aw2 = B.linear("add_embedding.linear_2.weight"); float* ab2 = B.f32("add_embedding.linear_2.bias");
            u->d_add_in = (float*)u->dmalloc((size_t)R * in * sizeof(float));
            u->d_add_h = (float*)u->dmalloc((size_t)R * temb_dim * sizeof(float));
            u->d_aug = (float*)u->dmalloc((size_t)R * temb_dim * sizeof(float));
            u->ctx_plan.push_back([=](hipStream_t s, int) { return cfgpp_op_f16_to_f32_rows(uu->ctx_text, uu->d_add_in, uu->ctx_cond_rows, pooled, in, 0, s); });
            u->ctx_plan.push_back([=](hipStream_t s, int) {
                for (int r = 0; r < uu->ctx_cond_rows; ++r) {
                    int e = cfgpp_op_sinusoid(uu->ctx_tids + (long)r * 6, 0.f, uu->d_add_in + (long)r * in + pooled, 6, tdim, tdim, 0, s);
                    if (e) return e;
                }
                return 0;
            });
            u->ctx_plan.push_back([=](hipStream_t s, int) { return cfgpp_op_skinny_gemm(uu->d_add_in, in, aw1, ab1, nullptr, 0, uu->d_add_h, temb_dim, uu->ctx_cond_rows, temb_dim, in, 0, 1, s); });
            u->ctx_plan.push_back([=](hipStream_t s, int) { return cfgpp_op_skinny_gemm(uu->d_add_h, temb_dim, aw2, ab2, nullptr, 0, uu->d_aug, temb_dim, uu->ctx_cond_rows, temb_dim, temb_dim, 0, 0, s); });
        }
    }

    auto load_res = [&](const std::string& p, int cin, int cout) {
        ResW w{}; w.cin = cin; w.cout = cout;
        w.n1g = B.f32(p + ".norm1.weight"); w.n1b = B.f32(p + ".norm1.bias");
        w.w1 = B.conv3(p + ".conv1.weight"); w.b1 = B.f32(p + ".conv1.bias");
        w.n2g = B.f32(p + ".norm2.weight"); w.n2b = B.f32(p + ".norm2.bias");
        w.w2 = B.conv3(p + ".conv2.weight"); w.b2 = B.f32(p + ".conv2.bias");
        if (cin != cout) { w.wsc = B.linear(p + ".conv_shortcut.weight"); w.bsc = B.f32(p + ".conv_shortcut.bias"); }
        w.temb_off = temb_off[p];
        return w;
    };
    auto resblock = [&](const std::string& p, const Tensor& x0, const Tensor* x1, int cout) {
        const int cin = x0.C + (x1 ? x1->C : 0);
        ResW w = load_res(p, cin, cout);
        Tensor g1 = u->acq(x0.H, x0.W, cin);
        P.groupnorm(x0, x1, g1.p, true, w.n1g, w.n1b, 1e-5f, true);
        Tensor h1 = u->acq(x0.H, x0.W, cout);
        P.conv3x3(g1, h1, w.w1, w.b1, 1, u->d_temb_all + w.temb_off, temb_ld, nullptr);
        u->rel(g1);
        Tensor g2 = u->acq(x0.H, x0.W, cout);
        P.groupnorm(h1, nullptr, g2.p, true, w.n2g, w.n2b, 1e-5f, true);
        u->rel(h1);
        Tensor out = u->acq(x0.H, x0.W, cout);
        if (cin != cout) {
            Tensor sc = u->acq(x0.H, x0.W, cout);
            P.conv1x1(x0, x1, sc, w.wsc, w.bsc);
            P.conv3x3(g2, out, w.w2, w.b2, 1, nullptr, 0, &sc);
            u->rel(sc);
        } else {
            P.conv3x3(g2, out, w.w2, w.b2, 1, nullptr, 0, &x0);
        }
        u->rel(g2);
        return out;
    };
    int cross_block_counter = 0;
    auto transformer = [&](const std::string& p, const Tensor& x, int depth, int nheads, int lvl) {
        half_t* const HQ = u->hq[lvl]; half_t* const HK = u->hk[lvl]; half_t* const HVT = u->hvt[lvl];
        const int C = x.C, tok = x.H * x.W, d = C / nheads, dp = round_up(d, 32);
        const int q_pad = round_up(tok, 128), k_pad = round_up(tok, 64);
        const int ck_pad = round_up(u->ctx_tokens, 64);
        float* ng = B.f32(p + ".norm.weight"); float* nb = B.f32(p + ".norm.bias");
        half_t* wpi = B.linear(p + ".proj_in.weight"); float* bpi = B.f32(p + ".proj_in.bias");
        half_t* wpo = B.linear(p + ".proj_out.weight"); float* bpo = B.f32(p + ".proj_out.bias");
        P.groupnorm(x, nullptr, u->tok_ln, false, ng, nb, 1e-6f, false);
        P.linear(u->tok_ln, C, u->tok_x, C, wpi, bpi, nullptr, tok);
        for (int k = 0; k < depth; ++k) {
            const std::string b = p + ".transformer_blocks." + std::to_string(k);
            float* l1g = B.f32(b + ".norm1.weight"); float* l1b = B.f32(b + ".norm1.bias");
            float* l2g = B.f32(b + ".norm2.weight"); float* l2b = B.f32(b + ".norm2.bias");
            float* l3g = B.f32(b + ".norm3.weight"); float* l3b = B.f32(b + ".norm3.bias");
            half_t* wqkv = B.concat({b + ".attn1.to_q.weight", b + ".attn1.to_k.weight", b + ".attn1.to_v.weight"});
            half_t* wq2 = B.linear(b + ".attn2.to_q.weight");
            half_t* wff1 = nullptr; float* bff1 = nullptr;
            B.geglu(b + ".ff.net.0.proj", C, &wff1, &bff1);
            half_t* wo1 = B.linear(b + ".attn1.to_out.0.weight"); float* bo1 = B.f32(b + ".attn1.to_out.0.bias");
            half_t* wkv2 = B.concat({b + ".attn2.to_k.weight", b + ".attn2.to_v.weight"});
            half_t* wo2 = B.linear(b + ".attn2.to_out.0.weight"); float* bo2 = B.f32(b + ".attn2.to_out.0.bias");
            half_t* wff2 = B.linear(b + ".ff.net.2.weight"); float* bff2 = B.f32(b + ".ff.net.2.bias");
            half_t* ck = (half_t*)u->dmalloc((size_t)R * nheads * ck_pad * dp * 2);
            half_t* cvt = (half_t*)u->dmalloc((size_t)R * nheads * dp * ck_pad * 2);
            if (!ck || !cvt || cfgpp_op_attention_prepare_vt(cvt, R * nheads, d, ck_pad, nullptr)) { B.ok = false; B.err = "cross-attention K/V^T allocation failed"; }
            {
                cfgpp_unet* uu = u; const int Dc = c.cross_attention_dim; const int ckp = ck_pad;
                IGemmArgs a = base_args(u);
                a.C0 = Dc; a.amode = 0; a.w = wkv2; a.N = 2 * C; a.K = Dc; a.epi = EPI_HEADS;
                a.hq = nullptr; a.hk = ck; a.hvt = cvt; a.part0 = 1; a.part_width = C; a.head_dim = d; a.head_dim_pad = dp;
                a.heads = nheads; a.tok_pad = ckp; a.q_tok_pad = ckp;
                u->ctx_plan.push_back([a, uu](hipStream_t s, int) mutable {
                    IGemmArgs b2 = a; b2.a0 = uu->ctx_ehs; b2.rows_per_batch = uu->ctx_tokens; b2.M = uu->ctx_rows * uu->ctx_tokens;
                    return igemm_launch(b2, s);
                });
            }
            ++cross_block_counter;
            P.layernorm(u->tok_x, u->tok_ln, l1g, l1b, tok, C);
            P.heads(u->tok_ln, C, wqkv, 3 * C, tok, 0, C, nheads, HQ, HK, HVT, q_pad, k_pad);
            P.attention(HQ, HK, HVT, u->tok_attn, nheads, d, tok, tok, q_pad, k_pad);
            P.linear(u->tok_attn, C, u->tok_x, C, wo1, bo1, u->tok_x, tok);
            P.layernorm(u->tok_x, u->tok_ln, l2g, l2b, tok, C);
            P.heads(u->tok_ln, C, wq2, C, tok, 0, C, nheads, HQ, nullptr, nullptr, q_pad, k_pad);
            {
                cfgpp_unet* uu = u;
                u->attn_macs_per_row += 2.0 * (double)nheads * tok * 77 * d;
                half_t* hq = HQ; half_t* o = u->tok_attn;
                u->plan.push_back([=](hipStream_t s, int rows) {
                    return cfgpp_op_attention(hq, ck, cvt, o, rows, nheads, d, tok, uu->ctx_tokens, q_pad, ck_pad, s);
                });
                u->tag(1, 2.0 * (double)nheads * tok * 77 * d, "cross_attn heads=" + std::to_string(nheads) + " N=" + std::to_string(tok) + " d=" + std::to_string(d));
            }
            P.linear(u->tok_attn, C, u->tok_x, C, wo2, bo2, u->tok_x, tok);
            P.layernorm(u->tok_x, u->tok_ln, l3g, l3b, tok, C);
            P.linear(u->tok_ln, C, u->tok_ff, 8 * C, wff1, bff1, nullptr, tok, EPI_GEGLU);
            P.linear(u->tok_ff, 4 * C, u->tok_x, C, wff2, bff2, u->tok_x, tok);
        }
        Tensor out = u->acq(x.H, x.W, C);
        P.linear_to_padded(u->tok_x, C, out, wpo, bpo, x);
        return out;
    };

    int H = c.sample_h, W = c.sample_w;
    Tensor x = u->acq(H, W, c0);
    {
        HostParam* pw = B.get("conv_in.weight"); HostParam* pb = B.get("conv_in.bias");
        CFGPP_REQUIRE(pw && pb, "finalize: %s", B.err.c_str());
        const int Ci = c.in_channels;
        std::vector<float> r((size_t)9 * Ci * c0);
        for (int o = 0; o < c0; ++o) for (int i = 0; i < Ci; ++i) for (int t = 0; t < 9; ++t)
            r[(size_t)(t * Ci + i) * c0 + o] = pw->f[((size_t)o * Ci + i) * 9 + t];
        float* dw = B.upload(r); float* db = B.upload(pb->f);
        cfgpp_unet* uu = u; half_t* xp = x.p; const int HH = H, WW = W;
        if (u->control) {
            u->d_img_emb = (half_t*)u->dmalloc((size_t)R * (H + 2) * (W + 2) * c0 * sizeof(half_t));
            CFGPP_REQUIRE(u->d_img_emb, "finalize: hipMalloc failed");
            u->plan.push_back([=](hipStream_t s, int rows) {
                return cfgpp_op_conv_in_add(uu->in_z, uu->in_z_half, nullptr, 1, 0, uu->d_img_emb, uu->img_rows, xp, dw, db, rows,
                                            uu->in_z_rows, Ci, HH, WW, c0, s);
            });
        } else if (Ci > c.out_channels) {
            const int Cz = c.out_channels, Cc = Ci - Cz;
            u->d_cond = (half_t*)u->dmalloc((size_t)R * Cc * H * W * sizeof(half_t));
            CFGPP_REQUIRE(u->d_cond, "finalize: hipMalloc failed");
            u->plan.push_back([=](hipStream_t s, int rows) {
                return cfgpp_op_conv_in_cond(uu->in_z, uu->in_z_half, uu->d_cond, uu->cond_rows, Cc, xp, dw, db, rows, uu->in_z_rows, Cz,
                                             HH, WW, c0, s);
            });
        } else {
            u->plan.push_back([=](hipStream_t s, int rows) {
                return cfgpp_op_conv_in(uu->in_z, uu->in_z_half, xp, dw, db, rows, uu->in_z_rows, Ci, HH, WW, c0, s);
            });
        }
    }
    std::vector<Tensor> skips; skips.push_back(x);
    for (int i = 0; i < L; ++i) {
        const int co = c.block_out_channels[i];
        const std::string p = "down_blocks." + std::to_string(i);
        for (int j = 0; j < c.layers_per_block; ++j) {
            Tensor y = resblock(p + ".resnets." + std::to_string(j), x, nullptr, co);
            if (c.level_has_attn[i]) {
                Tensor z = transformer(p + ".attentions." + std::to_string(j), y, c.transformer_depth[i], c.num_heads[i], i);
                u->rel(y); y = z;
            }
            x = y; skips.push_back(x);
        }
        if (i != L - 1) {
            half_t* wd = B.conv3(p + ".downsamplers.0.conv.weight"); float* bd = B.f32(p + ".downsamplers.0.conv.bias");
            H /= 2; W /= 2;
            Tensor y = u->acq(H, W, co);
            P.conv3x3(x, y, wd, bd, 2, nullptr, 0, nullptr);
            x = y; skips.push_back(x);
        }
    }
    {
        const int cm = c.block_out_channels[L - 1];
        Tensor y = resblock("mid_block.resnets.0", x, nullptr, cm);
        Tensor z = transformer("mid_block.attentions.0", y, c.transformer_depth[L - 1], c.num_heads[L - 1], L - 1);
        u->rel(y);
        Tensor w = resblock("mid_block.resnets.1", z, nullptr, cm);
        u->rel(z);
        x = w;
    }
    if (u->control) {
        int e = controlnet_tail(u, B, P, skips, x);
        if (e) return e;
        skips.clear();
        CFGPP_REQUIRE(B.ok, "finalize: %s", B.err.c_str());
        CFGPP_HIP_CHECK(hipDeviceSynchronize());
        u->plan_kind.resize(u->plan.size(), 3); u->plan_macs.resize(u->plan.size(), 0.0); u->plan_desc.resize(u->plan.size());
        u->finalized = true;
        return 0;
    }
    {
        u->ctrl_dst = skips; u->ctrl_dst.push_back(x);
        u->d_ctrl_tab = (CnAddEntry*)u->dmalloc(u->ctrl_dst.size() * sizeof(CnAddEntry));
        CFGPP_REQUIRE(u->d_ctrl_tab, "finalize: hipMalloc failed");
        for (const Tensor& t : u->ctrl_dst) u->ctrl_max_n8 = std::max(u->ctrl_max_n8, (long)R * t.H * t.W * (t.C / 8));
        cfgpp_unet* uu = u;
        const int n = (int)u->ctrl_dst.size();
        u->plan.push_back([uu, n](hipStream_t s, int rows) {
            if (!uu->ctrl || uu->ctrl_scale == 0.f) return 0;
            for (const Tensor& t : uu->ctrl_dst) if (t.gst_ok) *t.gst_ok = 0;
            return cn_residual_add_launch(uu->d_ctrl_tab, n, uu->ctrl_max_n8, rows, uu->ctrl_scale, s);
        });
        u->tag(3, 0.0, "controlnet residual add");
    }
    for (int i = 0; i < L; ++i) {
        const int lvl = L - 1 - i;
        const int co = c.block_out_channels[lvl];
        const std::string p = "up_blocks." + std::to_string(i);
        for (int j = 0; j < c.layers_per_block + 1; ++j) {
            Tensor skip = skips.back(); skips.pop_back();
            Tensor y = resblock(p + ".resnets." + std::to_string(j), x, &skip, co);
            u->rel(x); u->rel(skip);
            if (c.level_has_attn[lvl]) {
                Tensor z = transformer(p + ".attentions." + std::to_string(j), y, c.transformer_depth[lvl], c.num_heads[lvl], lvl);
                u->rel(y); y = z;
            }
            x = y;
        }
        if (i != L - 1) {
            half_t* wu = B.conv3(p + ".upsamplers.0.conv.weight"); float* bu = B.f32(p + ".upsamplers.0.conv.bias");
            H *= 2; W *= 2;
            Tensor y = u->acq(H, W, co);
            P.conv3x3(x, y, wu, bu, 3, nullptr, 0, nullptr);
            u->rel(x); x = y;
        }
    }
    {
        float* g = B.f32("conv_norm_out.weight"); float* b = B.f32("conv_norm_out.bias");
        Tensor gn = u->acq(H, W, c0);
        P.groupnorm(x, nullptr, gn.p, true, g, b, 1e-5f, true);
        HostParam* pw = B.get("conv_out.weight"); float* bo = B.f32("conv_out.bias");
        CFGPP_REQUIRE(pw, "finalize: %s", B.err.c_str());
        const int Co = c.out_channels;
        CFGPP_REQUIRE(Co <= 4, "finalize: out_channels %d > 4 unsupported", Co);
        std::vector<half_t> r((size_t)Co * 9 * c0);
        for (int o = 0; o < Co; ++o) for (int i = 0; i < c0; ++i) for (int t = 0; t < 9; ++t)
            r[((size_t)o * 9 + t) * c0 + i] = pw->h[((size_t)o * c0 + i) * 9 + t];
        half_t* dw = B.upload(r);
        cfgpp_unet* uu = u; half_t* gp = gn.p; const int HH = H, WW = W;
        u->macs_per_row += (double)H * W * Co * 9.0 * c0 + (double)c.sample_h * c.sample_w * c0 * 9.0 * c.in_channels;
        u->plan.push_back([=](hipStream_t s, int rows) { return cfgpp_op_conv_out(gp, uu->out_eps, 1, dw, bo, rows, HH, WW, c0, Co, s); });
    }
    CFGPP_REQUIRE(B.ok, "finalize: %s", B.err.c_str());
    CFGPP_REQUIRE(skips.empty(), "finalize: internal error, %d skips left", (int)skips.size());
    CFGPP_HIP_CHECK(hipDeviceSynchronize());
    u->plan_kind.resize(u->plan.size(), 3); u->plan_macs.resize(u->plan.size(), 0.0); u->plan_desc.resize(u->plan.size());
    u->finalized = true;
    return 0;
}

int cfgpp_unet_set_context(cfgpp_unet* u, const void* ehs, int rows, int tokens, const void* text_embeds,
                           const void* time_ids, int cond_rows, void* stream) {
    CFGPP_REQUIRE(u && u->finalized, "set_context: context not finalized");
    CFGPP_REQUIRE(ehs && rows > 0 && rows <= u->cfg.max_rows, "set_context: rows=%d (max %d)", rows, u->cfg.max_rows);
    CFGPP_REQUIRE(tokens == 77, "set_context: tokens=%d (the engine is built for 77 text tokens)", tokens);
    if (u->cfg.addition_embed) {
        CFGPP_REQUIRE(text_embeds && time_ids, "set_context: SDXL needs text_embeds and time_ids");
        CFGPP_REQUIRE(cond_rows == rows || cond_rows == 1, "set_context: cond_rows=%d must be rows (%d) or 1", cond_rows, rows);
    }
    u->ctx_ehs = (const half_t*)ehs; u->ctx_rows = rows; u->ctx_tokens = tokens;
    u->ctx_text = (const half_t*)text_embeds; u->ctx_tids = (const float*)time_ids; u->ctx_cond_rows = cond_rows;
    for (auto& op : u->ctx_plan) { int e = op((hipStream_t)stream, rows); if (e) return e; }
    u->ctx_set = true;
    return 0;
}

int cfgpp_unet_image_condition(cfgpp_unet* u, const void* cond, int cond_rows, void* stream) {
    CFGPP_REQUIRE(u && u->finalized, "image_condition: engine not finalized");
    if (u->control) {
        CFGPP_REQUIRE(cond && cond_rows > 0 && cond_rows <= u->cfg.max_rows, "image_condition: ControlNet image_rows=%d (1 .. %d)", cond_rows,
                      u->cfg.max_rows);
        u->img_in = cond; u->img_in_half = 1;
        for (auto& op : u->img_plan) { int e = op((hipStream_t)stream, cond_rows); if (e) return e; }
        u->img_in = nullptr;
        u->img_rows = cond_rows;
        return 0;
    }
    CFGPP_REQUIRE(u->cfg.in_channels > u->cfg.out_channels && u->d_cond,
                  "image_condition: this UNet takes %d input channels for %d latent channels - no image condition (not an inpaint UNet)",
                  u->cfg.in_channels, u->cfg.out_channels);
    CFGPP_REQUIRE(cond && cond_rows > 0 && cond_rows <= u->cfg.max_rows, "image_condition: cond_rows=%d (1 .. %d)", cond_rows, u->cfg.max_rows);
    const size_t bytes = (size_t)cond_rows * (u->cfg.in_channels - u->cfg.out_channels) * u->cfg.sample_h * u->cfg.sample_w * sizeof(half_t);
    CFGPP_HIP_CHECK(hipMemcpyAsync(u->d_cond, cond, bytes, hipMemcpyDeviceToDevice, (hipStream_t)stream));
    u->cond_rows = cond_rows;
    return 0;
}

int cfgpp_unet_attach_control(cfgpp_unet* u, cfgpp_unet* cn, float scale) {
    CFGPP_REQUIRE(u && u->finalized, "attach_control: UNet not finalized");
    CFGPP_REQUIRE(!u->control, "attach_control: the target is itself a ControlNet");
    if (!cn) { u->ctrl = nullptr; u->ctrl_scale = 0.f; return 0; }
    CFGPP_REQUIRE(cn->finalized && cn->control, "attach_control: not a finalized ControlNet (cfgpp_unet_create with out_channels = 0, then finalize)");
    const cfgpp_unet_config &a = u->cfg, &b = cn->cfg;
    CFGPP_REQUIRE(a.num_levels == b.num_levels && a.layers_per_block == b.layers_per_block, "attach_control: levels %d x %d vs the UNet's %d x %d",
                  b.num_levels, b.layers_per_block, a.num_levels, a.layers_per_block);
    for (int i = 0; i < a.num_levels; ++i)
        CFGPP_REQUIRE(a.block_out_channels[i] == b.block_out_channels[i], "attach_control: channels of level %d: %d vs the UNet's %d", i,
                      b.block_out_channels[i], a.block_out_channels[i]);
    CFGPP_REQUIRE(a.sample_h == b.sample_h && a.sample_w == b.sample_w, "attach_control: latent %d x %d vs the UNet's %d x %d", b.sample_h,
                  b.sample_w, a.sample_h, a.sample_w);
    CFGPP_REQUIRE(a.max_rows == b.max_rows, "attach_control: max_rows %d vs the UNet's %d", b.max_rows, a.max_rows);
    CFGPP_REQUIRE(b.in_channels == a.out_channels, "attach_control: the ControlNet takes %d latent channels, the UNet %d", b.in_channels,
                  a.out_channels);
    CFGPP_REQUIRE(cn->ctrl_res.size() == u->ctrl_dst.size(), "attach_control: %d residuals for %d skip connections + mid block",
                  (int)cn->ctrl_res.size(), (int)u->ctrl_dst.size());
    std::vector<CnAddEntry> tab(u->ctrl_dst.size());
    for (size_t i = 0; i < tab.size(); ++i) {
        const Tensor &d = u->ctrl_dst[i], &r = cn->ctrl_res[i];
        CFGPP_REQUIRE(d.H == r.H && d.W == r.W && d.C == r.C, "attach_control: residual %d is %d x %d x %d, the UNet tensor %d x %d x %d", (int)i,
                      r.H, r.W, r.C, d.H, d.W, d.C);
        tab[i] = CnAddEntry{d.p, r.p, d.H, d.W, d.C, 0};
    }
    CFGPP_HIP_CHECK(hipSetDevice(u->device));
    CFGPP_HIP_CHECK(hipDeviceSynchronize());
    CFGPP_HIP_CHECK(hipMemcpy(u->d_ctrl_tab, tab.data(), tab.size() * sizeof(CnAddEntry), hipMemcpyHostToDevice));
    u->ctrl = cn; u->ctrl_scale = scale;
    return 0;
}

int cfgpp_controlnet_residual(cfgpp_unet* cn, int i, float scale, float* out, int rows, int* hwc_out, void* stream) {
    CFGPP_REQUIRE(cn && cn->finalized && cn->control, "controlnet_residual: not a finalized ControlNet");
    const int n = (int)cn->ctrl_res.size();
    if (!out && !hwc_out) return n;
    CFGPP_REQUIRE(i >= 0 && i < n, "controlnet_residual: index %d (0 .. %d)", i, n - 1);
    const Tensor& r = cn->ctrl_res[i];
    if (hwc_out) { hwc_out[0] = r.H; hwc_out[1] = r.W; hwc_out[2] = r.C; }
    if (!out) return n;
    CFGPP_REQUIRE(rows > 0 && rows <= cn->cfg.max_rows, "controlnet_residual: rows=%d", rows);
    int e = cfgpp_op_residual_nchw(r.p, out, rows, r.H, r.W, r.C, scale, stream);
    return e ? e : n;
}

int cfgpp_unet_forward(cfgpp_unet* u, const void* z, int z_is_half, int z_rows, float t, void* eps_out, int rows,
                       void* stream) {
    CFGPP_REQUIRE(u && u->finalized, "forward: context not finalized");
    CFGPP_REQUIRE(u->ctx_set, "forward: set_context has not been called");
    CFGPP_REQUIRE(z && eps_out && z_rows > 0 && rows > 0 && rows <= u->cfg.max_rows, "forward: bad args (rows=%d max=%d)", rows, u->cfg.max_rows);
    CFGPP_REQUIRE(rows == u->ctx_rows, "forward: rows=%d but context was set for %d rows", rows, u->ctx_rows);
    CFGPP_REQUIRE(u->control || u->cfg.in_channels == u->cfg.out_channels || (u->cond_rows > 0 && (u->cond_rows == 1 || u->cond_rows == z_rows)),
                  "forward: inpaint UNet (%d input channels) needs cfgpp_unet_image_condition with 1 or z_rows=%d rows first (has %d)",
                  u->cfg.in_channels, z_rows, u->cond_rows);
    CFGPP_REQUIRE(!u->control || u->img_rows > 0, "forward: ControlNet without a control image (call cfgpp_unet_image_condition first)");
    if (u->ctrl && u->ctrl_scale != 0.f) {
        cfgpp_unet* cn = u->ctrl;
        CFGPP_REQUIRE(cn->img_rows > 0, "forward: a ControlNet is attached but has no control image (cfgpp_unet_image_condition)");
        CFGPP_REQUIRE(cn->ctx_set && cn->ctx_rows == rows, "forward: the attached ControlNet's context is set for %d rows, the forward runs %d",
                      cn->ctx_set ? cn->ctx_rows : 0, rows);
        int e = cfgpp_unet_forward(cn, z, z_is_half, z_rows, t, eps_out, rows, stream);
        if (e) return e;
    }
    u->in_z = z; u->in_z_half = z_is_half; u->in_z_rows = z_rows; u->in_t = t; u->in_t_dev = nullptr; u->out_eps = eps_out;
    if (u->tuned_rows != rows && igemm_autotune_enabled()) {
        int e = u->tune_plan((hipStream_t)stream, rows); if (e) return e;
        ++u->tuned_serial;
    }
    for (auto& op : u->plan) { int e = op((hipStream_t)stream, rows); if (e) return e; }
    return 0;
}

int cfgpp_sample_graph_ddim(cfgpp_unet* u, void* z, void* z0t, int z_is_half, int z_rows, void* eps, const void* eps_uc,
                            const void* eps_c, int rows, const float* host_steps, int n_steps, float lam, int tweedie_uc,
                            int renoise_uc, void* stream) {
    CFGPP_REQUIRE(u && u->finalized && u->ctx_set, "sample_graph: context not ready");
    CFGPP_REQUIRE(z && z0t && eps && eps_uc && eps_c && host_steps && n_steps > 0 && z_rows > 0, "sample_graph: bad args");
    CFGPP_REQUIRE(rows == u->ctx_rows && rows <= u->cfg.max_rows, "sample_graph: rows=%d but context was set for %d rows", rows, u->ctx_rows);
    CFGPP_REQUIRE(!u->ctrl && !u->control, "sample_graph: a ControlNet is attached (a controlled step is not captured): detach it "
                                            "(cfgpp_unet_attach_control(u, NULL, 0)) or run the eager loop");
    hipStream_t s = (hipStream_t)stream;
    CFGPP_REQUIRE(u->cfg.in_channels == u->cfg.out_channels || (u->cond_rows > 0 && (u->cond_rows == 1 || u->cond_rows == z_rows)),
                  "sample_graph: inpaint UNet (%d input channels) needs cfgpp_unet_image_condition with 1 or z_rows=%d rows first (has %d)",
                  u->cfg.in_channels, z_rows, u->cond_rows);
    const long n = (long)z_rows * u->cfg.out_channels * u->cfg.sample_h * u->cfg.sample_w;
    if (!u->d_step_cur) {
        u->d_step_cur = (float*)u->dmalloc(8 * sizeof(float));
        u->d_step_idx = (int*)u->dmalloc(sizeof(int));
        CFGPP_REQUIRE(u->d_step_cur && u->d_step_idx, "sample_graph: out of device memory");
        CFGPP_HIP_CHECK(hipStreamCreateWithFlags(&u->cap_stream, hipStreamNonBlocking));
    }
    if (n_steps > u->step_tab_cap) {
        u->drop_graphs();
        const int cap = n_steps < 64 ? 64 : n_steps;
        u->d_step_tab = (float*)u->dmalloc((size_t)cap * 8 * sizeof(float));
        CFGPP_REQUIRE(u->d_step_tab, "sample_graph: out of device memory");
        u->step_tab_cap = cap;
    }
    const cfgpp_unet::GraphKey want{z, z0t, eps, eps_uc, eps_c, z_is_half, z_rows, rows, tweedie_uc, renoise_uc, lam, n, 0, u->cond_rows};
    auto same = [&](const cfgpp_unet::GraphKey& k) {
        return k.z == want.z && k.z0t == want.z0t && k.eps == want.eps && k.euc == want.euc && k.ec == want.ec && k.z_half == want.z_half &&
               k.z_rows == want.z_rows && k.rows == want.rows && k.tw == want.tw && k.rn == want.rn && k.lam == want.lam && k.n == want.n &&
               k.tuned_serial == u->tuned_serial && k.cond_rows == want.cond_rows;
    };
    int hit = -1;
    for (size_t i = 0; i < u->graphs.size(); ++i) if (same(u->graphs[i].key)) hit = (int)i;
    if (hit < 0) {
        int e = cfgpp_unet_forward(u, z, z_is_half, z_rows, host_steps[0], eps, rows, stream);
        if (e) return e;
        CFGPP_HIP_CHECK(hipStreamSynchronize(s));
        for (size_t i = 0; i < u->graphs.size();)
            if (u->graphs[i].key.tuned_serial != u->tuned_serial) { cfgpp_unet::destroy(u->graphs[i]); u->graphs.erase(u->graphs.begin() + i); } else ++i;
        cfgpp_unet::Graph g{want, nullptr, nullptr};
        g.key.tuned_serial = u->tuned_serial;
        u->in_t_dev = u->d_step_cur;
        hipError_t he = hipStreamBeginCapture(u->cap_stream, hipStreamCaptureModeRelaxed);
        int rc = 0;
        if (he == hipSuccess) {
            rc = step_advance_launch(u->d_step_tab, u->d_step_idx, u->d_step_cur, u->cap_stream);
            for (size_t i = 0; i < u->plan.size() && rc == 0; ++i) rc = u->plan[i](u->cap_stream, rows);
            if (rc == 0) rc = step_ddim_dev_launch(z, z0t, eps_uc, eps_c, 1, z_is_half, lam, u->d_step_cur + 1, tweedie_uc, renoise_uc, n, u->cap_stream);
            he = hipStreamEndCapture(u->cap_stream, &g.graph);
        }
        u->in_t_dev = nullptr;
        if (he != hipSuccess || rc != 0 || !g.graph) {
            cfgpp_unet::destroy(g);
            if (rc == 0) cfgpp_set_error("sample_graph: stream capture failed: %s", hipGetErrorString(he));
            return rc ? rc : -1;
        }
        he = hipGraphInstantiate(&g.exec, g.graph, nullptr, nullptr, 0);
        if (he != hipSuccess) { cfgpp_unet::destroy(g); cfgpp_set_error("sample_graph: hipGraphInstantiate: %s", hipGetErrorString(he)); return -1; }
        if (u->graphs.size() >= 4) { cfgpp_unet::destroy(u->graphs.front()); u->graphs.erase(u->graphs.begin()); }
        u->graphs.push_back(g);
        hit = (int)u->graphs.size() - 1;
    }
    if (hit != (int)u->graphs.size() - 1) std::swap(u->graphs[hit], u->graphs.back());
    hipGraphExec_t exec = u->graphs.back().exec;
    std::vector<float> tab((size_t)n_steps * 8, 0.f);
    for (int i = 0; i < n_steps; ++i) for (int k = 0; k < 5; ++k) tab[(size_t)i * 8 + k] = host_steps[(size_t)i * 5 + k];
    CFGPP_HIP_CHECK(hipMemcpyAsync(u->d_step_tab, tab.data(), tab.size() * sizeof(float), hipMemcpyHostToDevice, s));
    CFGPP_HIP_CHECK(hipStreamSynchronize(s));
    CFGPP_HIP_CHECK(hipMemsetAsync(u->d_step_idx, 0, sizeof(int), s));
    for (int i = 0; i < n_steps; ++i) CFGPP_HIP_CHECK(hipGraphLaunch(exec, s));
    return 0;
}

int cfgpp_unet_profile(cfgpp_unet* u, const void* z, int z_is_half, int z_rows, float t, void* eps_out, int rows,
                       void* stream, double* out_ms, double* out_flops, int* out_launches, char* detail, long detail_cap) {
    CFGPP_REQUIRE(u && u->finalized && u->ctx_set, "profile: context not ready");
    CFGPP_REQUIRE(z && eps_out && out_ms && out_flops && out_launches && rows == u->ctx_rows, "profile: bad args");
    u->in_z = z; u->in_z_half = z_is_half; u->in_z_rows = z_rows; u->in_t = t; u->out_eps = eps_out;
    hipStream_t s = (hipStream_t)stream;
    const size_t n = u->plan.size();
    std::vector<hipEvent_t> ev(n + 1);
    for (auto& e : ev) CFGPP_HIP_CHECK(hipEventCreate(&e));
    CFGPP_HIP_CHECK(hipEventRecord(ev[0], s));
    int rc = 0;
    for (size_t i = 0; i < n && rc == 0; ++i) { rc = u->plan[i](s, rows); if (rc == 0 && hipEventRecord(ev[i + 1], s) != hipSuccess) rc = -1; }
    if (rc == 0 && hipStreamSynchronize(s) != hipSuccess) rc = -1;
    for (int k = 0; k < 4; ++k) { out_ms[k] = 0; out_flops[k] = 0; out_launches[k] = 0; }
    if (rc == 0) {
        for (size_t i = 0; i < n; ++i) {
            float ms = 0.f; hipEventElapsedTime(&ms, ev[i], ev[i + 1]);
            const int k = u->plan_kind[i];
            out_ms[k] += ms; out_flops[k] += 2.0 * u->plan_macs[i] * rows; out_launches[k] += 1;
        }
        if (detail && detail_cap > 0) {
            std::string txt;
            for (size_t i = 0; i < n; ++i) {
                float ms = 0.f; hipEventElapsedTime(&ms, ev[i], ev[i + 1]);
                char line[256];
                snprintf(line, sizeof(line), "%zu\t%d\t%s\t%.1f\t%.3f\n", i, u->plan_kind[i], u->plan_desc[i].c_str(), ms * 1e3,
                         2.0 * u->plan_macs[i] * rows * 1e-9);
                txt += line;
            }
            const long ncopy = std::min<long>((long)txt.size(), detail_cap - 1);
            std::memcpy(detail, txt.data(), ncopy); detail[ncopy] = 0;
        }
    }
    for (auto& e : ev) hipEventDestroy(e);
    return rc;
}

int cfgpp_unet_tuning(cfgpp_unet* u, int rows, int* hints, int cap, int set) {
    CFGPP_REQUIRE(u && u->finalized && hints && rows > 0, "unet_tuning: bad args");
    const int n = (int)u->cfg_hints.size();
    CFGPP_REQUIRE(cap >= n, "unet_tuning: buffer of %d for %d launches", cap, n);
    if (set) {
        u->tuned_by_rows[rows] = std::vector<int>(hints, hints + n);
        if (u->tuned_rows == rows) u->tuned_rows = 0;
        ++u->tuned_serial;
        return n;
    }
    auto it = u->tuned_by_rows.find(rows);
    if (it == u->tuned_by_rows.end()) { cfgpp_set_error("unet_tuning: batch %d has not been tuned", rows); return -3; }
    std::copy(it->second.begin(), it->second.end(), hints);
    return n;
}

double cfgpp_unet_flops(cfgpp_unet* u, int rows) {
    if (!u || !u->finalized) return 0.0;
    return 2.0 * (u->macs_per_row + u->attn_macs_per_row) * rows;
}
double cfgpp_unet_device_bytes(cfgpp_unet* u) { return u ? u->dev_bytes : 0.0; }

static float* g_op_gstat = nullptr;
static int g_op_gstat_flag = 0;
void cfgpp_op_igemm_set_gstat(void* buf) { g_op_gstat = (float*)buf; }
int cfgpp_op_igemm_gstat_written() { return g_op_gstat_flag; }

int cfgpp_op_igemm(const void* a0, const void* a1, int C0, int C1, int taps, int amode, int H, int W,
                   const void* w, int M, int N, const float* bias, const float* temb, int temb_ld,
                   const void* resid, int rmode, int rld, void* out, int omode, int old_, int epi, void* stream) {
    IGemmArgs a = base_args();
    a.a0 = (const half_t*)a0; a.a1 = (const half_t*)a1; a.C0 = C0; a.C1 = C1; a.taps = taps; a.amode = amode; a.H = H; a.W = W;
    a.w = (const half_t*)w; a.M = M; a.N = N; a.K = taps * (C0 + C1); a.bias = bias; a.temb = temb; a.temb_ld = temb_ld;
    a.rows_per_batch = H * W; a.resid = (const half_t*)resid; a.rmode = rmode; a.rld = rld;
    a.out = (half_t*)out; a.omode = omode; a.old = old_; a.epi = epi;
    a.gstat = g_op_gstat; a.stat_flag = &g_op_gstat_flag; g_op_gstat_flag = 0;
    return igemm_launch(a, (hipStream_t)stream);
}

int cfgpp_op_igemm_heads(const void* a_, int K, const void* w, int M, int N, const float* bias, int rows_per_batch,
                         void* hq, void* hk, void* hvt, int part0, int part_width, int head_dim, int heads,
                         int q_tok_pad, int tok_pad, void* stream) {
    IGemmArgs a = base_args();
    a.a0 = (const half_t*)a_; a.C0 = K; a.amode = 0; a.w = (const half_t*)w; a.M = M; a.N = N; a.K = K; a.bias = bias;
    a.epi = EPI_HEADS; a.rows_per_batch = rows_per_batch; a.hq = (half_t*)hq; a.hk = (half_t*)hk; a.hvt = (half_t*)hvt;
    a.part0 = part0; a.part_width = part_width; a.head_dim = head_dim; a.head_dim_pad = round_up(head_dim, 32);
    a.heads = heads; a.q_tok_pad = q_tok_pad; a.tok_pad = tok_pad;
    return igemm_launch(a, (hipStream_t)stream);
}

}
```

### cfgpp_amd/engine.py

```python
from __future__ import annotations

import ctypes as C
from typing import Dict, Iterable, Optional, Tuple

import torch

from . import _lib
from ._lib import CfgppError, UNetConfigC, check
from .unet_config import UNetConfig


def _require_cuda(t: torch.Tensor, name: str):
    if not t.is_cuda:
        raise CfgppError(f"{name} must live on the GPU (got {t.device}); the HIP path has no CPU fallback")
    if not t.is_contiguous():
        raise CfgppError(f"{name} must be contiguous")


def _stream_ptr(t: Optional[torch.Tensor] = None) -> int:
    if t is not None and t.is_cuda:
        return torch.cuda.current_stream(t.device).cuda_stream
    return torch.cuda.current_stream().cuda_stream


def _ptr(t: Optional[torch.Tensor]) -> Optional[int]:
    return None if t is None else t.data_ptr()


def step_ddim(z: torch.Tensor, z0t_out: torch.Tensor, eps_uc: torch.Tensor, eps_c: torch.Tensor,
              lam: float, coeffs: Tuple[float, float, float, float], tweedie_uc: bool, renoise_uc: bool):
    lib = _lib.load()
    for n, t in (("z", z), ("z0t_out", z0t_out), ("eps_uc", eps_uc), ("eps_c", eps_c)):
        _require_cuda(t, n)
    if z.dtype != z0t_out.dtype or z.dtype not in (torch.float16, torch.float32):
        raise CfgppError("step_ddim: z and z0t_out must both be fp32 or both fp16")
    if eps_uc.dtype != eps_c.dtype or eps_uc.dtype not in (torch.float16, torch.float32):
        raise CfgppError("step_ddim: eps must both be fp16 or both fp32")
    if not (z.numel() == z0t_out.numel() == eps_uc.numel() == eps_c.numel()):
        raise CfgppError("step_ddim: size mismatch")
    c1, c2, c3, c4 = (float(x) for x in coeffs)
    if z.dtype == torch.float16:
        if eps_uc.dtype != torch.float16:
            raise CfgppError("step_ddim: an fp16 latent needs fp16 eps")
        check(lib.cfgpp_step_ddim_h(z.data_ptr(), z0t_out.data_ptr(), eps_uc.data_ptr(), eps_c.data_ptr(), float(lam),
                                    c1, c2, c3, c4, int(bool(tweedie_uc)), int(bool(renoise_uc)), z.numel(), _stream_ptr(z)),
              "cfgpp_step_ddim_h")
        return
    check(lib.cfgpp_step_ddim(z.data_ptr(), z0t_out.data_ptr(), eps_uc.data_ptr(), eps_c.data_ptr(),
                              1 if eps_uc.dtype == torch.float16 else 0, float(lam), c1, c2, c3, c4,
                              int(bool(tweedie_uc)), int(bool(renoise_uc)), z.numel(), _stream_ptr(z)),
          "cfgpp_step_ddim")


def step_ddim_masked(z: torch.Tensor, z0t_out: torch.Tensor, eps_uc: torch.Tensor, eps_c: torch.Tensor, lam: float,
                     coeffs: Tuple[float, float, float, float], tweedie_uc: bool, renoise_uc: bool, mask: torch.Tensor,
                     src: torch.Tensor, noise: torch.Tensor, a: float, b: float):
    lib = _lib.load()
    for n, t in (("z", z), ("z0t_out", z0t_out), ("eps_uc", eps_uc), ("eps_c", eps_c), ("mask", mask), ("src", src),
                 ("noise", noise)):
        _require_cuda(t, n)
    if z.dtype != torch.float32 or z0t_out.dtype != torch.float32 or noise.dtype != torch.float32:
        raise CfgppError("step_ddim_masked: z, z0t_out and noise must be fp32")
    if eps_uc.dtype != torch.float16 or eps_c.dtype != torch.float16 or src.dtype != torch.float16:
        raise CfgppError("step_ddim_masked: eps and src must be fp16")
    if mask.dtype not in (torch.bool, torch.uint8):
        raise CfgppError("step_ddim_masked: mask must be bool or uint8 (binarized)")
    if z.dim() != 4 or tuple(z.shape[1:2]) != (4,):
        raise CfgppError(f"step_ddim_masked: z shape {tuple(z.shape)} is not [B, 4, h, w]")
    B, hw = int(z.shape[0]), int(z.shape[2]) * int(z.shape[3])
    for n, t in (("z0t_out", z0t_out), ("eps_uc", eps_uc), ("eps_c", eps_c), ("src", src), ("noise", noise)):
        if tuple(t.shape) != tuple(z.shape):
            raise CfgppError(f"step_ddim_masked: {n} shape {tuple(t.shape)} != z shape {tuple(z.shape)}")
    if mask.numel() != B * hw:
        raise CfgppError(f"step_ddim_masked: mask has {mask.numel()} elements for B={B} x hw={hw}")
    c1, c2, c3, c4 = (float(x) for x in coeffs)
    check(lib.cfgpp_step_ddim_masked(z.data_ptr(), z0t_out.data_ptr(), eps_uc.data_ptr(), eps_c.data_ptr(), float(lam), c1, c2, c3, c4,
                                     int(bool(tweedie_uc)), int(bool(renoise_uc)), mask.data_ptr(), src.data_ptr(), noise.data_ptr(),
                                     float(a), float(b), B, hw, _stream_ptr(z)), "cfgpp_step_ddim_masked")


def kdiff_input(x: torch.Tensor, xc_out: torch.Tensor, s: float, mode: int):
    lib = _lib.load()
    _require_cuda(x, "x")
    _require_cuda(xc_out, "xc_out")
    if x.dtype != torch.float16 or xc_out.dtype != torch.float16:
        raise CfgppError("kdiff_input: fp16 latents expected")
    check(lib.cfgpp_kdiff_input(x.data_ptr(), xc_out.data_ptr(), float(s), int(mode), x.numel(), _stream_ptr(x)),
          "cfgpp_kdiff_input")


def step_kdiff(x: torch.Tensor, den_out: torch.Tensor, old: Optional[torch.Tensor], eps_uc: torch.Tensor,
               eps_c: torch.Tensor, coef9, variant: int, xl_form: bool, euler_branch: bool, write_old: bool):
    lib = _lib.load()
    for n, t in (("x", x), ("den_out", den_out), ("eps_uc", eps_uc), ("eps_c", eps_c)):
        _require_cuda(t, n)
        if t.dtype != torch.float16:
            raise CfgppError(f"step_kdiff: {n} must be fp16")
    if old is not None:
        _require_cuda(old, "old")
    arr = (C.c_float * 9)(*[float(v) for v in coef9])
    check(lib.cfgpp_step_kdiff(x.data_ptr(), den_out.data_ptr(), _ptr(old), eps_uc.data_ptr(), eps_c.data_ptr(),
                               arr, int(variant), int(bool(xl_form)), int(bool(euler_branch)), int(bool(write_old)),
                               x.numel(), _stream_ptr(x)), "cfgpp_step_kdiff")


def kdiff_denoise(x, eps_uc, eps_c, lam: float, sigma: float, den_out, uden_out):
    lib = _lib.load()
    for n, t in (("x", x), ("eps_uc", eps_uc), ("eps_c", eps_c), ("den_out", den_out), ("uden_out", uden_out)):
        _require_cuda(t, n)
        if t.dtype != torch.float16:
            raise CfgppError(f"kdiff_denoise: {n} must be fp16")
    check(lib.cfgpp_kdiff_denoise(x.data_ptr(), eps_uc.data_ptr(), eps_c.data_ptr(), float(lam), float(sigma),
                                  den_out.data_ptr(), uden_out.data_ptr(), x.numel(), _stream_ptr(x)), "cfgpp_kdiff_denoise")


def lincomb(out, x, y, z, a: float, b: float, mode: int):
    lib = _lib.load()
    for n, t in (("out", out), ("x", x), ("y", y)) + ((("z", z),) if z is not None else ()):
        _require_cuda(t, n)
        if t.dtype != torch.float16:
            raise CfgppError(f"lincomb: {n} must be fp16")
    check(lib.cfgpp_lincomb(out.data_ptr(), x.data_ptr(), y.data_ptr(), _ptr(z), float(a), float(b), int(mode), x.numel(),
                            _stream_ptr(x)), "cfgpp_lincomb")


def unet_config_c(cfg: UNetConfig, H: int, W: int, max_rows: int, out_channels: Optional[int] = None) -> UNetConfigC:
    cc = UNetConfigC()
    cc.in_channels = cfg.in_channels
    cc.out_channels = cfg.out_channels if out_channels is None else int(out_channels)
    cc.num_levels = cfg.num_levels
    for i in range(cfg.num_levels):
        cc.block_out_channels[i] = cfg.block_out_channels[i]
        cc.level_has_attn[i] = cfg.level_has_attn[i]
        cc.transformer_depth[i] = cfg.transformer_depth[i]
        cc.num_heads[i] = cfg.num_heads[i]
    cc.layers_per_block = cfg.layers_per_block
    cc.cross_attention_dim = cfg.cross_attention_dim
    cc.addition_embed = cfg.addition_embed
    cc.addition_time_embed_dim = cfg.addition_time_embed_dim
    cc.addition_pooled_dim = cfg.addition_pooled_dim
    cc.norm_groups = cfg.norm_groups
    cc.sample_h, cc.sample_w = int(H), int(W)
    cc.max_rows = int(max_rows)
    return cc


class HipUNet:

    def __init__(self, cfg: UNetConfig, max_rows: int, sample_hw: Optional[Tuple[int, int]] = None,
                 device: int = 0):
        self.lib = _lib.load()
        if not torch.cuda.is_available():
            raise CfgppError("HipUNet needs a ROCm GPU (torch.cuda.is_available() is False); "
                             "there is no CPU fallback for the HIP path")
        self.cfg = cfg
        self.device = int(device)
        self.max_rows = int(max_rows)
        H, W = sample_hw if sample_hw is not None else (cfg.sample_size, cfg.sample_size)
        self.H, self.W = int(H), int(W)
        cc = unet_config_c(cfg, self.H, self.W, self.max_rows)
        self._h = self.lib.cfgpp_unet_create(C.byref(cc), self.device)
        if not self._h:
            raise CfgppError("cfgpp_unet_create failed: " + _lib.last_error())
        self._keep = {}
        self.finalized = False
        self.latent_channels = cfg.out_channels
        self.cond_channels = cfg.in_channels - cfg.out_channels

    def __del__(self):
        h = getattr(self, "_h", None)
        if h:
            try:
                torch.cuda.synchronize()
            except Exception:
                pass
            self.lib.cfgpp_unet_destroy(h)
            self._h = None

    def load_tensor(self, key: str, t: torch.Tensor):
        t = t.detach().cpu().contiguous()
        if t.dtype == torch.float16:
            dt = 1
        else:
            t = t.to(torch.float32)
            dt = 0
        shape = (C.c_long * t.dim())(*t.shape)
        check(self.lib.cfgpp_unet_load_tensor(self._h, key.encode(), t.data_ptr(), dt, shape, t.dim()),
              f"cfgpp_unet_load_tensor({key})")

    def load_state_dict(self, items: Iterable[Tuple[str, torch.Tensor]]):
        if isinstance(items, dict):
            items = items.items()
        for k, v in items:
            self.load_tensor(k, v)
        return self

    def finalize(self):
        check(self.lib.cfgpp_unet_finalize(self._h), "cfgpp_unet_finalize")
        self.finalized = True
        return self

    def set_context(self, ehs: torch.Tensor, text_embeds: Optional[torch.Tensor] = None,
                    time_ids: Optional[torch.Tensor] = None):
        dev = torch.device("cuda", self.device)
        ehs = ehs.to(device=dev, dtype=torch.float16).contiguous()
        rows, tokens = int(ehs.shape[0]), int(ehs.shape[1])
        te = ti = None
        cond_rows = 0
        if self.cfg.addition_embed:
            if text_embeds is None or time_ids is None:
                raise CfgppError("set_context: SDXL needs text_embeds and time_ids")
            te = text_embeds.to(device=dev, dtype=torch.float16).contiguous()
            ti = time_ids.to(device=dev, dtype=torch.float32).contiguous()
            cond_rows = int(te.shape[0])
            if int(ti.shape[0]) != cond_rows:
                raise CfgppError("set_context: text_embeds / time_ids row mismatch")
        self._keep["ctx"] = (ehs, te, ti)
        self.rows = rows
        check(self.lib.cfgpp_unet_set_context(self._h, ehs.data_ptr(), rows, tokens, _ptr(te), _ptr(ti), cond_rows,
                                              _stream_ptr(ehs)), "cfgpp_unet_set_context")

    def image_condition(self, cond: torch.Tensor):
        if self.cond_channels <= 0:
            raise CfgppError(f"image_condition: {self.cfg.name} takes no image condition (in_channels == out_channels)")
        dev = torch.device("cuda", self.device)
        cond = cond.to(device=dev, dtype=torch.float16).contiguous()
        if cond.dim() != 4 or tuple(cond.shape[1:]) != (self.cond_channels, self.H, self.W):
            raise CfgppError(f"image_condition: cond shape {tuple(cond.shape)} != [*, {self.cond_channels}, {self.H}, {self.W}]")
        check(self.lib.cfgpp_unet_image_condition(self._h, cond.data_ptr(), int(cond.shape[0]), _stream_ptr(cond)),
              "cfgpp_unet_image_condition")
        self._keep["cond"] = cond

    def forward(self, z: torch.Tensor, t: float, eps_out: Optional[torch.Tensor] = None) -> torch.Tensor:
        _require_cuda(z, "z")
        if z.dtype not in (torch.float16, torch.float32):
            raise CfgppError("forward: z must be fp16 or fp32")
        zr = int(z.shape[0])
        if tuple(z.shape[1:]) != (self.latent_channels, self.H, self.W):
            raise CfgppError(f"forward: z shape {tuple(z.shape)} != [*, {self.latent_channels}, {self.H}, {self.W}]")
        rows = self.rows
        if rows % zr != 0:
            raise CfgppError(f"forward: rows={rows} is not a multiple of z rows={zr}")
        if eps_out is None:
            eps_out = torch.empty((rows, self.cfg.out_channels, self.H, self.W), dtype=torch.float16, device=z.device)
        check(self.lib.cfgpp_unet_forward(self._h, z.data_ptr(), 1 if z.dtype == torch.float16 else 0, zr, float(t),
                                          eps_out.data_ptr(), rows, _stream_ptr(z)), "cfgpp_unet_forward")
        return eps_out

    def attach_control(self, cn, scale: float):
        check(self.lib.cfgpp_unet_attach_control(self._h, None if cn is None else cn._h, float(scale)), "cfgpp_unet_attach_control")
        self._keep["control"] = cn

    def sample_graph_ddim(self, z: torch.Tensor, z0t: torch.Tensor, eps: torch.Tensor, eps_uc: torch.Tensor, eps_c: torch.Tensor,
                          steps, lam: float, tweedie_uc: bool, renoise_uc: bool):
        for n, t in (("z", z), ("z0t", z0t), ("eps", eps)):
            _require_cuda(t, n)
        if z.dtype != z0t.dtype or z.dtype not in (torch.float16, torch.float32) or eps.dtype != torch.float16:
            raise CfgppError("sample_graph_ddim: z / z0t must both be fp32 or both fp16, eps fp16")
        if tuple(z.shape[1:]) != (self.latent_channels, self.H, self.W) or z.shape != z0t.shape:
            raise CfgppError(f"sample_graph_ddim: z shape {tuple(z.shape)}")
        if int(eps.shape[0]) != self.rows or self.rows % int(z.shape[0]) != 0:
            raise CfgppError(f"sample_graph_ddim: eps rows {int(eps.shape[0])} / z rows {int(z.shape[0])} vs context rows {self.rows}")
        flat = [float(v) for st in steps for v in st]
        if len(flat) != 5 * len(steps) or not steps:
            raise CfgppError("sample_graph_ddim: steps must be a non-empty list of (t, c1, c2, c3, c4)")
        arr = (C.c_float * len(flat))(*flat)
        check(self.lib.cfgpp_sample_graph_ddim(self._h, z.data_ptr(), z0t.data_ptr(), 1 if z.dtype == torch.float16 else 0, int(z.shape[0]),
                                               eps.data_ptr(), eps_uc.data_ptr(), eps_c.data_ptr(), self.rows, arr, len(steps), float(lam),
                                               int(bool(tweedie_uc)), int(bool(renoise_uc)), _stream_ptr(z)), "cfgpp_sample_graph_ddim")

    def profile(self, z: torch.Tensor, t: float, detail: bool = False) -> dict:
        _require_cuda(z, "z")
        rows = self.rows
        eps = torch.empty((rows, self.cfg.out_channels, self.H, self.W), dtype=torch.float16, device=z.device)
        ms, fl, ln = (C.c_double * 4)(), (C.c_double * 4)(), (C.c_int * 4)()
        buf = C.create_string_buffer(1 << 20) if detail else None
        check(self.lib.cfgpp_unet_profile(self._h, z.data_ptr(), 1 if z.dtype == torch.float16 else 0, int(z.shape[0]),
                                          float(t), eps.data_ptr(), rows, _stream_ptr(z), ms, fl, ln, buf, (1 << 20) if detail else 0),
              "cfgpp_unet_profile")
        names = ("igemm", "attention", "norm", "small")
        out = {n: dict(ms=ms[i], flops=fl[i], launches=ln[i]) for i, n in enumerate(names)}
        if detail:
            out["detail"] = buf.value.decode()
        return out

    def export_tuning(self, rows: Optional[int] = None):
        rows = self.rows if rows is None else int(rows)
        buf = (C.c_int * 4096)()
        n = self.lib.cfgpp_unet_tuning(self._h, rows, buf, 4096, 0)
        if n < 0:
            raise CfgppError("cfgpp_unet_tuning: " + _lib.last_error())
        return [int(buf[i]) for i in range(n)]

    def import_tuning(self, hints, rows: int):
        buf = (C.c_int * len(hints))(*[int(h) for h in hints])
        n = self.lib.cfgpp_unet_tuning(self._h, int(rows), buf, len(hints), 1)
        if n < 0:
            raise CfgppError("cfgpp_unet_tuning: " + _lib.last_error())

    def flops(self, rows: int) -> float:
        return float(self.lib.cfgpp_unet_flops(self._h, int(rows)))

    def device_bytes(self) -> float:
        return float(self.lib.cfgpp_unet_device_bytes(self._h))
```

### cfgpp_amd/hip_engine.py

```python
from __future__ import annotations

import os
from typing import Optional, Tuple

import torch

from . import engine as E
from . import _lib
from ._lib import CfgppError
from .tune_cache import PinCache, build_id
from .unet_config import CONFIGS, UNetConfig
from .weights import load_safetensors_iter, synth_state_dict_iter


class HipEngine:

    def __init__(self, cfg: UNetConfig, max_batch: int = 1, latent_hw: Optional[Tuple[int, int]] = None,
                 device=None, weights="synthetic", weight_seed: int = 0):
        if isinstance(cfg, str):
            cfg = CONFIGS[cfg]
        if not torch.cuda.is_available():
            raise CfgppError("HipEngine needs a ROCm GPU; the HIP path has no CPU fallback")
        dev = torch.device(device if device is not None else "cuda")
        if dev.type != "cuda":
            raise CfgppError(f"HipEngine cannot run on device '{dev}': the HIP path has no CPU fallback")
        self.device = torch.device("cuda", dev.index if dev.index is not None else torch.cuda.current_device())
        self.cfg = cfg
        self.max_batch = int(max_batch)
        torch.cuda.set_device(self.device)
        self.unet = E.HipUNet(cfg, max_rows=2 * self.max_batch, sample_hw=latent_hw, device=self.device.index)
        if weights == "synthetic":
            items = synth_state_dict_iter(cfg, weight_seed)
        elif isinstance(weights, str):
            items = load_safetensors_iter(weights)
        else:
            items = weights.items() if isinstance(weights, dict) else weights
        self.unet.load_state_dict(items).finalize()
        self.H, self.W = self.unet.H, self.unet.W
        self._pins = PinCache(getattr(cfg, "name", type(cfg).__name__), (self.H, self.W), torch.cuda.get_device_properties(self.device).name,
                              build_id(_lib.LIB_PATH), lambda rows: self.unet.export_tuning(rows), lambda h, rows: self.unet.import_tuning(h, rows),
                              knobs=lambda: (int(self.unet.lib.cfgpp_igemm_tuner_state()),))
        self._ctx_key = None
        self._ctx = None
        self._control = None
        self._eps = None
        self._g_buf = None
        self.check_finite = os.environ.get("CFGPP_CHECK_FINITE", "0") not in ("", "0")

    def _finite_or_raise(self, t):
        if not bool(torch.isfinite(self._eps).all()):
            bad = int((~torch.isfinite(self._eps)).sum())
            raise CfgppError(f"UNet output at t={t} holds {bad} non-finite values (fp16 overflow inside the UNet?) - CFGPP_CHECK_FINITE")

    def set_context(self, uc: torch.Tensor, c: torch.Tensor, text_embeds=None, time_ids=None):
        B = max(int(uc.shape[0]), int(c.shape[0]))
        if B > self.max_batch:
            raise CfgppError(f"batch {B} exceeds engine max_batch {self.max_batch}")
        if uc.shape[0] != B:
            uc = uc.expand(B, -1, -1)
        if c.shape[0] != B:
            c = c.expand(B, -1, -1)
        ehs = torch.cat([uc, c], dim=0)
        self.unet.set_context(ehs, text_embeds, time_ids)
        self._ctx = (ehs, text_embeds, time_ids)
        if self._control is not None:
            self._control[0].set_context(ehs, text_embeds, time_ids)
        self._pins.load(2 * B)
        self.B = B
        if self._eps is None or int(self._eps.shape[0]) != 2 * B:
            self._eps = torch.empty((2 * B, self.cfg.out_channels, self.H, self.W), dtype=torch.float16, device=self.device)

    def image_condition(self, cond: torch.Tensor):
        self.unet.image_condition(cond)

    def set_control(self, cn, image: torch.Tensor, scale: float = 1.0):
        cn.set_image(image)
        if self._ctx is not None:
            cn.set_context(*self._ctx)
        self.unet.attach_control(cn, float(scale))
        self._control = (cn, float(scale))

    def clear_control(self):
        if self._control is not None:
            self.unet.attach_control(None, 0.0)
        self._control = None

    def build_controlnet(self, spec, seed: int = 0):
        from .controlnet import build_controlnet
        return build_controlnet(spec, self.cfg, 2 * self.max_batch, (self.H, self.W), self.device.index, seed)

    @property
    def control(self):
        return self._control

    def predict(self, z: torch.Tensor, t: float):
        eps = self.unet.forward(z, float(t), self._eps)
        self._pins.save(self.unet.rows)
        if self.check_finite:
            self._finite_or_raise(t)
        return eps[: self.B], eps[self.B:]

    @property
    def graph_enabled(self) -> bool:
        return os.environ.get("CFGPP_GRAPH", "0") not in ("", "0") and self._control is None

    def ddim_loop_graph(self, zt: torch.Tensor, steps, lam: float, tweedie_uc: bool, renoise_uc: bool, single: str = ""):
        key = (int(zt.shape[0]), zt.dtype)
        if self._g_buf is None or self._g_buf[0] != key:
            self._g_buf = (key, torch.empty_like(zt), torch.empty_like(zt))
        _, gz, gz0 = self._g_buf
        gz.copy_(zt)
        eps = self._eps
        euc, ec = eps[: self.B], eps[self.B:]
        if single == "uc":
            ec = euc
        elif single == "c":
            euc = ec
        self.unet.sample_graph_ddim(gz, gz0, eps, euc, ec, steps, lam, tweedie_uc, renoise_uc)
        self._pins.save(self.unet.rows)
        if self.check_finite:
            self._finite_or_raise(steps[-1][0])
        return gz0.clone(), gz.clone()

    def export_tuning(self):
        return self.unet.export_tuning(self.unet.rows)

    def import_tuning(self, hints, batch: int):
        self.unet.import_tuning(hints, 2 * int(batch))
        self._pins.mark_imported(2 * int(batch))

    def device_bytes(self) -> float:
        return self.unet.device_bytes()

    step_ddim = staticmethod(E.step_ddim)
    step_ddim_masked = staticmethod(E.step_ddim_masked)
    kdiff_input = staticmethod(E.kdiff_input)
    step_kdiff = staticmethod(E.step_kdiff)
    kdiff_denoise = staticmethod(E.kdiff_denoise)
    lincomb = staticmethod(E.lincomb)

    def randn_like(self, x):
        return torch.randn_like(x)

    def flops_per_forward(self, rows: int) -> float:
        return self.unet.flops(rows)
```

### cfgpp_amd/tune_cache.py

```python
from __future__ import annotations

import hashlib
import json
import os
import re
import tempfile
from typing import Callable, List, Optional

_BUILD_ID = {}


def build_id(lib_path: str) -> str:
    if lib_path not in _BUILD_ID:
        h = hashlib.sha1()
        try:
            with open(lib_path, "rb") as f:
                for chunk in iter(lambda: f.read(1 << 20), b""):
                    h.update(chunk)
            _BUILD_ID[lib_path] = h.hexdigest()[:12]
        except OSError:
            _BUILD_ID[lib_path] = "nolib"
    return _BUILD_ID[lib_path]


def skewed_run() -> bool:
    return any(k.startswith(("ROCP_", "ROCPROFILER_", "ROCPROF_")) or k == "HSA_TOOLS_LIB" for k in os.environ)


def cache_dir() -> Optional[str]:
    d = os.environ.get("CFGPP_TUNE_CACHE", os.path.join(os.path.expanduser("~"), ".cache", "cfgpp_amd"))
    if d in ("", "0") or os.environ.get("CFGPP_AUTOTUNE", "1") == "0":
        return None
    return d


class PinCache:

    def __init__(self, model: str, latent_hw, device_name: str, build: str,
                 export_fn: Callable[[int], List[int]], import_fn: Callable[[List[int], int], None], directory: Optional[str] = None,
                 knobs: Optional[Callable[[], tuple]] = None):
        self.dir = cache_dir() if directory is None else directory
        self.tag = "_".join(re.sub(r"[^A-Za-z0-9.]+", "-", str(x)) for x in (model, f"{latent_hw[0]}x{latent_hw[1]}"))
        self.dev = re.sub(r"[^A-Za-z0-9.]+", "-", device_name)
        self.build = build
        self._export, self._import = export_fn, import_fn
        self._done = set()
        self._tries = {}
        self._knobs = knobs
        self._knobs_default = knobs() if knobs is not None else None

    def path(self, rows: int) -> str:
        return os.path.join(self.dir, f"tune_{self.tag}_r{rows}_{self.dev}_{self.build}.json")

    def load(self, rows: int) -> bool:
        if self.dir is None or rows in self._done:
            return False
        try:
            with open(self.path(rows)) as f:
                rec = json.load(f)
            hints = [int(h) for h in rec["hints"]]
            if rec.get("rows") != rows or not hints:
                return False
            self._import(hints, rows)
        except Exception:
            return False
        self._done.add(rows)
        return True

    def mark_imported(self, rows: int):
        self._done.add(rows)

    def save(self, rows: int) -> bool:
        if self.dir is None or rows in self._done:
            return False
        if skewed_run() or (self._knobs is not None and self._knobs() != self._knobs_default):
            self._done.add(rows)
            return False
        try:
            hints = self._export(rows)
        except Exception:
            hints = None
        if not hints:
            self._tries[rows] = self._tries.get(rows, 0) + 1
            if self._tries[rows] >= 3:
                self._done.add(rows)
            return False
        try:
            os.makedirs(self.dir, exist_ok=True)
            fd, tmp = tempfile.mkstemp(dir=self.dir, prefix=".tune_", suffix=".tmp")
            with os.fdopen(fd, "w") as f:
                json.dump({"rows": rows, "hints": hints, "model": self.tag, "device": self.dev, "build": self.build}, f)
            os.replace(tmp, self.path(rows))
            self._done.add(rows)
            return True
        except Exception:
            self._done.add(rows)
            return False
```

Before: 8.673 images/sec.

## Share CFG-invariant UNet prefix across uncond/cond rows and fan out

```diff
diff --git a/cfgpp_amd/_lib.py b/cfgpp_amd/_lib.py
--- a/cfgpp_amd/_lib.py
+++ b/cfgpp_amd/_lib.py
@@ -84,6 +84,9 @@
     "cfgpp_op_igemm_gstat_written": (_I, []),
     "cfgpp_groupnorm_set_prestats": (None, [_I]),
     "cfgpp_groupnorm_prestats_enabled": (_I, []),
+    "cfgpp_unet_set_share_prefix": (None, [_I]),
+    "cfgpp_unet_share_prefix_enabled": (_I, []),
+    "cfgpp_unet_shared_prefix_ops": (_I, [_P, _I, _I]),
     "cfgpp_op_layernorm": (_I, [_P, _P, _P, _P, _L, _I, _F, _P]),
     "cfgpp_op_attention_prepare_vt": (_I, [_P, _I, _I, _I, _P]),
     "cfgpp_op_attention": (_I, [_P, _P, _P, _P, _I, _I, _I, _I, _I, _I, _I, _P]),
diff --git a/cfgpp_amd/csrc/cfgpp_debug.h b/cfgpp_amd/csrc/cfgpp_debug.h
--- a/cfgpp_amd/csrc/cfgpp_debug.h
+++ b/cfgpp_amd/csrc/cfgpp_debug.h
@@ -18,6 +18,9 @@
 int cfgpp_op_igemm_gstat_written(void);
 void cfgpp_groupnorm_set_prestats(int on);
 int cfgpp_groupnorm_prestats_enabled(void);
+void cfgpp_unet_set_share_prefix(int on);
+int cfgpp_unet_share_prefix_enabled(void);
+int cfgpp_unet_shared_prefix_ops(cfgpp_unet* u, int rows, int z_rows);
 void cfgpp_groupnorm_set_mode(int mode);
 int cfgpp_op_layernorm(const void* x, void* y, const float* gamma, const float* beta, long rows, int C,
                        float eps, void* stream);
diff --git a/cfgpp_amd/csrc/common.h b/cfgpp_amd/csrc/common.h
--- a/cfgpp_amd/csrc/common.h
+++ b/cfgpp_amd/csrc/common.h
@@ -40,6 +40,8 @@
     int H, W, C, pad_;
 };
 int cn_residual_add_launch(const CnAddEntry* tab, int n, long max_n8, int rows, float scale, hipStream_t s);
+
+int fanout_rows_launch(half_t* const* p, const long* row_elems, int nseg, int h, hipStream_t s);
 
 static inline int cdiv(long a, long b) { return (int)((a + b - 1) / b); }
 
diff --git a/cfgpp_amd/csrc/engine_base.h b/cfgpp_amd/csrc/engine_base.h
--- a/cfgpp_amd/csrc/engine_base.h
+++ b/cfgpp_amd/csrc/engine_base.h
@@ -6,6 +6,7 @@
 #include <functional>
 #include <map>
 #include <string>
+#include <utility>
 #include <vector>
 
 #include "../../include/cfgpp.h"
@@ -47,6 +48,12 @@
     std::vector<int> plan_kind;
     std::vector<double> plan_macs;
     std::vector<std::string> plan_desc;
+    std::vector<char> plan_share;
+    int rows_for(size_t i, int rows, bool shared) const {
+        const int m = i < plan_share.size() ? plan_share[i] : 0;
+        if (m == 0) return rows;
+        return shared ? rows / 2 : (m == 1 ? rows : 0);
+    }
     void tag(int kind, double macs, const std::string& desc = "") {
         plan_kind.resize(plan.size(), 3); plan_macs.resize(plan.size(), 0.0); plan_desc.resize(plan.size());
         if (!plan.empty()) { plan_kind.back() = kind; plan_macs.back() = macs; plan_desc.back() = desc; }
@@ -54,19 +61,21 @@
     std::deque<int> cfg_hints;
     std::vector<int*> plan_hint;
     int tuned_rows = 0;
-    std::map<int, std::vector<int>> tuned_by_rows;
+    bool tuned_shared = false;
+    std::map<std::pair<int, bool>, std::vector<int>> tuned_by_rows;
     int* new_hint(bool in_main_plan) {
         cfg_hints.push_back(0);
         int* h = &cfg_hints.back();
         if (in_main_plan) { plan_hint.resize(plan.size() + 1, nullptr); plan_hint[plan.size()] = h; }
         return h;
     }
-    int tune_plan(hipStream_t s, int rows) {
-        auto cached = tuned_by_rows.find(rows);
+    int tune_plan(hipStream_t s, int rows, bool shared = false) {
+        const auto key = std::make_pair(rows, shared);
+        auto cached = tuned_by_rows.find(key);
         if (cached != tuned_by_rows.end() && cached->second.size() == cfg_hints.size()) {
             size_t k = 0;
             for (int& h : cfg_hints) h = cached->second[k++];
-            tuned_rows = rows;
+            tuned_rows = rows; tuned_shared = shared;
             return 0;
         }
         static const int cands[] = {0, 1, 4, 5, 6, 7, 8, 9, 10, 11, 12, 13, 14, 15, 16, 17, 20, 24, 25, 26, 27, 28};
@@ -85,7 +94,7 @@
             for (int rep = 0; rep < 2 && rc == 0; ++rep) {
                 if (hipEventRecord(ev[0], s) != hipSuccess) rc = -1;
                 for (size_t i = 0; i < n && rc == 0; ++i) {
-                    rc = plan[i](s, rows);
+                    rc = plan[i](s, rows_for(i, rows, shared));
                     if (plan_hint[i]) applied[i] = (char)igemm_last_hint_applied();
                     if (rc == 0 && hipEventRecord(ev[i + 1], s) != hipSuccess) rc = -1;
                 }
@@ -118,8 +127,8 @@
         for (int& h : cfg_hints) h = 0;
         for (size_t i = 0; i < n; ++i) if (plan_hint[i]) *plan_hint[i] = bestc[i];
         for (auto& e : ev) hipEventDestroy(e);
-        if (rc == 0) tuned_by_rows[rows] = std::vector<int>(cfg_hints.begin(), cfg_hints.end());
-        tuned_rows = rows;
+        if (rc == 0) tuned_by_rows[key] = std::vector<int>(cfg_hints.begin(), cfg_hints.end());
+        tuned_rows = rows; tuned_shared = shared;
         return rc;
     }
     std::map<std::tuple<int, int, int>, std::vector<std::pair<half_t*, float*>>> pool;
diff --git a/cfgpp_amd/csrc/small_kernels.hip b/cfgpp_amd/csrc/small_kernels.hip
--- a/cfgpp_amd/csrc/small_kernels.hip
+++ b/cfgpp_amd/csrc/small_kernels.hip
@@ -1,3 +1,5 @@
+#include <algorithm>
+
 #include "common.h"
 
 namespace {
@@ -252,6 +254,41 @@
     }
 }
 
+struct FanoutArgs {
+    uint4* p[3];
+    long n16[3];
+};
+
+__global__ void __launch_bounds__(256)
+fanout_rows_kernel(FanoutArgs a) {
+    const long n = a.n16[blockIdx.y];
+    const uint4* __restrict__ src = a.p[blockIdx.y];
+    uint4* __restrict__ dst = a.p[blockIdx.y] + n;
+    const long T = (long)gridDim.x * 256;
+    long i = (long)blockIdx.x * 256 + threadIdx.x;
+    for (; i + 3 * T < n; i += 4 * T) {
+        const uint4 v0 = src[i], v1 = src[i + T], v2 = src[i + 2 * T], v3 = src[i + 3 * T];
+        dst[i] = v0; dst[i + T] = v1; dst[i + 2 * T] = v2; dst[i + 3 * T] = v3;
+    }
+    for (; i < n; i += T) dst[i] = src[i];
+}
+
+}
+
+int fanout_rows_launch(half_t* const* p, const long* row_elems, int nseg, int h, hipStream_t s) {
+    CFGPP_REQUIRE(p && row_elems && nseg > 0 && nseg <= 3 && h > 0, "fanout_rows: bad args");
+    FanoutArgs a{};
+    long most = 0;
+    for (int k = 0; k < nseg; ++k) {
+        CFGPP_REQUIRE(p[k] && row_elems[k] > 0 && row_elems[k] % 8 == 0 && ((uintptr_t)p[k] & 15) == 0, "fanout_rows: segment %d is not made of 16-byte units", k);
+        a.p[k] = reinterpret_cast<uint4*>(p[k]);
+        a.n16[k] = (long)h * (row_elems[k] / 8);
+        most = std::max(most, a.n16[k]);
+    }
+    dim3 grid((unsigned)std::min<long>(cdiv(most, 256 * 4), 2048), (unsigned)nseg);
+    hipLaunchKernelGGL(fanout_rows_kernel, grid, dim3(256), 0, s, a);
+    CFGPP_HIP_CHECK(hipGetLastError());
+    return 0;
 }
 
 
diff --git a/cfgpp_amd/csrc/unet.hip b/cfgpp_amd/csrc/unet.hip
--- a/cfgpp_amd/csrc/unet.hip
+++ b/cfgpp_amd/csrc/unet.hip
@@ -15,6 +15,15 @@
     struct Graph { GraphKey key; hipGraph_t graph; hipGraphExec_t exec; };
     std::vector<Graph> graphs;
     int tuned_serial = 0;
+    int prefix_ops = 0;
+    double prefix_macs_per_row = 0;
+    int ran_shared = -1;
+    bool shares(int rows, int z_rows) const;
+    bool enter_call(int rows, int z_rows) {
+        const bool sh = shares(rows, z_rows);
+        if (ran_shared != (int)sh) { if (ran_shared >= 0) ++tuned_serial; ran_shared = (int)sh; }
+        return sh;
+    }
     static void destroy(Graph& g) { if (g.exec) hipGraphExecDestroy(g.exec); if (g.graph) hipGraphDestroy(g.graph); g.exec = nullptr; g.graph = nullptr; }
     void drop_graphs() { for (auto& g : graphs) destroy(g); graphs.clear(); }
     ~cfgpp_unet() { drop_graphs(); if (cap_stream) hipStreamDestroy(cap_stream); }
@@ -40,6 +49,9 @@
     cfgpp_unet* ctrl = nullptr; float ctrl_scale = 0.f;
     CnAddEntry* d_ctrl_tab = nullptr; long ctrl_max_n8 = 0;
 };
+
+static int g_share_prefix = 1;
+bool cfgpp_unet::shares(int rows, int z_rows) const { return g_share_prefix && prefix_ops > 0 && rows == 2 * z_rows; }
 
 namespace {
 
@@ -419,6 +431,7 @@
         return out;
     };
     int cross_block_counter = 0;
+    long prefix_from = -1;
     auto transformer = [&](const std::string& p, const Tensor& x, int depth, int nheads, int lvl) {
         half_t* const HQ = u->hq[lvl]; half_t* const HK = u->hk[lvl]; half_t* const HVT = u->hvt[lvl];
         const int C = x.C, tok = x.H * x.W, d = C / nheads, dp = round_up(d, 32);
@@ -463,6 +476,23 @@
             P.linear(u->tok_attn, C, u->tok_x, C, wo1, bo1, u->tok_x, tok);
             P.layernorm(u->tok_x, u->tok_ln, l2g, l2b, tok, C);
             P.heads(u->tok_ln, C, wq2, C, tok, 0, C, nheads, HQ, nullptr, nullptr, q_pad, k_pad);
+            if (prefix_from >= 0) {
+                u->plan_share.assign(u->plan.size(), 0);
+                for (size_t i = (size_t)prefix_from; i < u->plan.size(); ++i) {
+                    u->plan_share[i] = 1; ++u->prefix_ops;
+                    if (i < u->plan_macs.size()) u->prefix_macs_per_row += u->plan_macs[i];
+                }
+                half_t* const fp0 = u->tok_x; half_t* const fp1 = HQ; half_t* const fp2 = x.p;
+                const long fe0 = (long)tok * C, fe1 = (long)nheads * q_pad * dp, fe2 = (long)(x.H + 2) * (x.W + 2) * C;
+                u->plan.push_back([=](hipStream_t s, int h) {
+                    if (h <= 0) return 0;
+                    half_t* const fp[3] = {fp0, fp1, fp2}; const long fe[3] = {fe0, fe1, fe2};
+                    return fanout_rows_launch(fp, fe, 3, h, s);
+                });
+                u->plan_share.push_back(2);
+                u->tag(3, 0.0, "cfg fan-out tok_x + HQ + resid HW=" + std::to_string(tok) + " C=" + std::to_string(C));
+                prefix_from = -1;
+            }
             {
                 cfgpp_unet* uu = u;
                 u->attn_macs_per_row += 2.0 * (double)nheads * tok * 77 * d;
@@ -519,6 +549,7 @@
         const int co = c.block_out_channels[i];
         const std::string p = "down_blocks." + std::to_string(i);
         for (int j = 0; j < c.layers_per_block; ++j) {
+            if (i == 0 && j == 0 && !per_row_temb && c.level_has_attn[0]) prefix_from = (long)u->plan.size();
             Tensor y = resblock(p + ".resnets." + std::to_string(j), x, nullptr, co);
             if (c.level_has_attn[i]) {
                 Tensor z = transformer(p + ".attentions." + std::to_string(j), y, c.transformer_depth[i], c.num_heads[i], i);
@@ -550,6 +581,7 @@
         CFGPP_REQUIRE(B.ok, "finalize: %s", B.err.c_str());
         CFGPP_HIP_CHECK(hipDeviceSynchronize());
         u->plan_kind.resize(u->plan.size(), 3); u->plan_macs.resize(u->plan.size(), 0.0); u->plan_desc.resize(u->plan.size());
+        u->plan_share.resize(u->plan.size(), 0);
         u->finalized = true;
         return 0;
     }
@@ -609,6 +641,7 @@
     CFGPP_REQUIRE(skips.empty(), "finalize: internal error, %d skips left", (int)skips.size());
     CFGPP_HIP_CHECK(hipDeviceSynchronize());
     u->plan_kind.resize(u->plan.size(), 3); u->plan_macs.resize(u->plan.size(), 0.0); u->plan_desc.resize(u->plan.size());
+    u->plan_share.resize(u->plan.size(), 0);
     u->finalized = true;
     return 0;
 }
@@ -714,11 +747,12 @@
         if (e) return e;
     }
     u->in_z = z; u->in_z_half = z_is_half; u->in_z_rows = z_rows; u->in_t = t; u->in_t_dev = nullptr; u->out_eps = eps_out;
-    if (u->tuned_rows != rows && igemm_autotune_enabled()) {
-        int e = u->tune_plan((hipStream_t)stream, rows); if (e) return e;
+    const bool shared = u->enter_call(rows, z_rows);
+    if ((u->tuned_rows != rows || u->tuned_shared != shared) && igemm_autotune_enabled()) {
+        int e = u->tune_plan((hipStream_t)stream, rows, shared); if (e) return e;
         ++u->tuned_serial;
     }
-    for (auto& op : u->plan) { int e = op((hipStream_t)stream, rows); if (e) return e; }
+    for (size_t i = 0; i < u->plan.size(); ++i) { int e = u->plan[i]((hipStream_t)stream, u->rows_for(i, rows, shared)); if (e) return e; }
     return 0;
 }
 
@@ -748,6 +782,7 @@
         CFGPP_REQUIRE(u->d_step_tab, "sample_graph: out of device memory");
         u->step_tab_cap = cap;
     }
+    u->enter_call(rows, z_rows);
     const cfgpp_unet::GraphKey want{z, z0t, eps, eps_uc, eps_c, z_is_half, z_rows, rows, tweedie_uc, renoise_uc, lam, n, 0, u->cond_rows};
     auto same = [&](const cfgpp_unet::GraphKey& k) {
         return k.z == want.z && k.z0t == want.z0t && k.eps == want.eps && k.euc == want.euc && k.ec == want.ec && k.z_half == want.z_half &&
@@ -769,7 +804,8 @@
         int rc = 0;
         if (he == hipSuccess) {
             rc = step_advance_launch(u->d_step_tab, u->d_step_idx, u->d_step_cur, u->cap_stream);
-            for (size_t i = 0; i < u->plan.size() && rc == 0; ++i) rc = u->plan[i](u->cap_stream, rows);
+            const bool shared = u->shares(rows, z_rows);
+            for (size_t i = 0; i < u->plan.size() && rc == 0; ++i) rc = u->plan[i](u->cap_stream, u->rows_for(i, rows, shared));
             if (rc == 0) rc = step_ddim_dev_launch(z, z0t, eps_uc, eps_c, 1, z_is_half, lam, u->d_step_cur + 1, tweedie_uc, renoise_uc, n, u->cap_stream);
             he = hipStreamEndCapture(u->cap_stream, &g.graph);
         }
@@ -803,26 +839,32 @@
     u->in_z = z; u->in_z_half = z_is_half; u->in_z_rows = z_rows; u->in_t = t; u->out_eps = eps_out;
     hipStream_t s = (hipStream_t)stream;
     const size_t n = u->plan.size();
+    const bool shared = u->enter_call(rows, z_rows);
+    std::vector<int> op_rows(n);
+    for (size_t i = 0; i < n; ++i) op_rows[i] = u->rows_for(i, rows, shared);
     std::vector<hipEvent_t> ev(n + 1);
     for (auto& e : ev) CFGPP_HIP_CHECK(hipEventCreate(&e));
     CFGPP_HIP_CHECK(hipEventRecord(ev[0], s));
     int rc = 0;
-    for (size_t i = 0; i < n && rc == 0; ++i) { rc = u->plan[i](s, rows); if (rc == 0 && hipEventRecord(ev[i + 1], s) != hipSuccess) rc = -1; }
+    for (size_t i = 0; i < n && rc == 0; ++i) { rc = u->plan[i](s, op_rows[i]); if (rc == 0 && hipEventRecord(ev[i + 1], s) != hipSuccess) rc = -1; }
     if (rc == 0 && hipStreamSynchronize(s) != hipSuccess) rc = -1;
     for (int k = 0; k < 4; ++k) { out_ms[k] = 0; out_flops[k] = 0; out_launches[k] = 0; }
     if (rc == 0) {
         for (size_t i = 0; i < n; ++i) {
+            if (op_rows[i] == 0) continue;
             float ms = 0.f; hipEventElapsedTime(&ms, ev[i], ev[i + 1]);
             const int k = u->plan_kind[i];
-            out_ms[k] += ms; out_flops[k] += 2.0 * u->plan_macs[i] * rows; out_launches[k] += 1;
+            out_ms[k] += ms; out_flops[k] += 2.0 * u->plan_macs[i] * op_rows[i]; out_launches[k] += 1;
         }
         if (detail && detail_cap > 0) {
             std::string txt;
             for (size_t i = 0; i < n; ++i) {
+                if (op_rows[i] == 0) continue;
                 float ms = 0.f; hipEventElapsedTime(&ms, ev[i], ev[i + 1]);
                 char line[256];
-                snprintf(line, sizeof(line), "%zu\t%d\t%s\t%.1f\t%.3f\n", i, u->plan_kind[i], u->plan_desc[i].c_str(), ms * 1e3,
-                         2.0 * u->plan_macs[i] * rows * 1e-9);
+                const std::string desc = u->plan_desc[i] + (op_rows[i] != rows ? " rows=" + std::to_string(op_rows[i]) : std::string());
+                snprintf(line, sizeof(line), "%zu\t%d\t%s\t%.1f\t%.3f\n", i, u->plan_kind[i], desc.c_str(), ms * 1e3,
+                         2.0 * u->plan_macs[i] * op_rows[i] * 1e-9);
                 txt += line;
             }
             const long ncopy = std::min<long>((long)txt.size(), detail_cap - 1);
@@ -838,12 +880,12 @@
     const int n = (int)u->cfg_hints.size();
     CFGPP_REQUIRE(cap >= n, "unet_tuning: buffer of %d for %d launches", cap, n);
     if (set) {
-        u->tuned_by_rows[rows] = std::vector<int>(hints, hints + n);
+        for (int sh = 0; sh < 2; ++sh) u->tuned_by_rows[std::make_pair(rows, sh != 0)] = std::vector<int>(hints, hints + n);
         if (u->tuned_rows == rows) u->tuned_rows = 0;
         ++u->tuned_serial;
         return n;
     }
-    auto it = u->tuned_by_rows.find(rows);
+    auto it = u->tuned_by_rows.find(std::make_pair(rows, u->ran_shared == 1));
     if (it == u->tuned_by_rows.end()) { cfgpp_set_error("unet_tuning: batch %d has not been tuned", rows); return -3; }
     std::copy(it->second.begin(), it->second.end(), hints);
     return n;
@@ -851,7 +893,15 @@
 
 double cfgpp_unet_flops(cfgpp_unet* u, int rows) {
     if (!u || !u->finalized) return 0.0;
-    return 2.0 * (u->macs_per_row + u->attn_macs_per_row) * rows;
+    const double once = u->ran_shared == 1 ? u->prefix_macs_per_row * (rows / 2) : 0.0;
+    return 2.0 * ((u->macs_per_row + u->attn_macs_per_row) * rows - once);
+}
+
+void cfgpp_unet_set_share_prefix(int on) { g_share_prefix = on ? 1 : 0; }
+int cfgpp_unet_share_prefix_enabled(void) { return g_share_prefix; }
+int cfgpp_unet_shared_prefix_ops(cfgpp_unet* u, int rows, int z_rows) {
+    if (!u || !u->finalized) return 0;
+    return u->shares(rows, z_rows) ? u->prefix_ops : 0;
 }
 double cfgpp_unet_device_bytes(cfgpp_unet* u) { return u ? u->dev_bytes : 0.0; }
 
diff --git a/cfgpp_amd/engine.py b/cfgpp_amd/engine.py
--- a/cfgpp_amd/engine.py
+++ b/cfgpp_amd/engine.py
@@ -301,5 +301,16 @@
     def flops(self, rows: int) -> float:
         return float(self.lib.cfgpp_unet_flops(self._h, int(rows)))
 
+    def shared_prefix_ops(self, rows: int, z_rows: int) -> int:
+        return int(self.lib.cfgpp_unet_shared_prefix_ops(self._h, int(rows), int(z_rows)))
+
     def device_bytes(self) -> float:
         return float(self.lib.cfgpp_unet_device_bytes(self._h))
+
+
+def set_share_prefix(on: bool):
+    _lib.load().cfgpp_unet_set_share_prefix(1 if on else 0)
+
+
+def share_prefix_enabled() -> bool:
+    return bool(_lib.load().cfgpp_unet_share_prefix_enabled())
diff --git a/cfgpp_amd/hip_engine.py b/cfgpp_amd/hip_engine.py
--- a/cfgpp_amd/hip_engine.py
+++ b/cfgpp_amd/hip_engine.py
@@ -39,7 +39,8 @@
         self.H, self.W = self.unet.H, self.unet.W
         self._pins = PinCache(getattr(cfg, "name", type(cfg).__name__), (self.H, self.W), torch.cuda.get_device_properties(self.device).name,
                               build_id(_lib.LIB_PATH), lambda rows: self.unet.export_tuning(rows), lambda h, rows: self.unet.import_tuning(h, rows),
-                              knobs=lambda: (int(self.unet.lib.cfgpp_igemm_tuner_state()),))
+                              knobs=lambda: (int(self.unet.lib.cfgpp_igemm_tuner_state()),),
+                              mode=lambda rows: "shared" if self.unet.shared_prefix_ops(rows, rows // 2) else "")
         self._ctx_key = None
         self._ctx = None
         self._control = None
diff --git a/cfgpp_amd/tune_cache.py b/cfgpp_amd/tune_cache.py
--- a/cfgpp_amd/tune_cache.py
+++ b/cfgpp_amd/tune_cache.py
@@ -38,7 +38,7 @@
 
     def __init__(self, model: str, latent_hw, device_name: str, build: str,
                  export_fn: Callable[[int], List[int]], import_fn: Callable[[List[int], int], None], directory: Optional[str] = None,
-                 knobs: Optional[Callable[[], tuple]] = None):
+                 knobs: Optional[Callable[[], tuple]] = None, mode: Optional[Callable[[int], str]] = None):
         self.dir = cache_dir() if directory is None else directory
         self.tag = "_".join(re.sub(r"[^A-Za-z0-9.]+", "-", str(x)) for x in (model, f"{latent_hw[0]}x{latent_hw[1]}"))
         self.dev = re.sub(r"[^A-Za-z0-9.]+", "-", device_name)
@@ -48,9 +48,11 @@
         self._tries = {}
         self._knobs = knobs
         self._knobs_default = knobs() if knobs is not None else None
+        self._mode = mode
 
     def path(self, rows: int) -> str:
-        return os.path.join(self.dir, f"tune_{self.tag}_r{rows}_{self.dev}_{self.build}.json")
+        mode = self._mode(rows) if self._mode is not None else ""
+        return os.path.join(self.dir, f"tune_{self.tag}_r{rows}_{self.dev}_{self.build}{'_' + mode if mode else ''}.json")
 
     def load(self, rows: int) -> bool:
         if self.dir is None or rows in self._done:
```

After: 8.866 images/sec, median of 6. +2.2%, better.
